# FumiyukiKato/FL-TEE

Hardware: AMD Instinct MI355X
Metric: aggregated params/sec (device-resident), 100 clients x MLP-MNIST updates (higher is better)
Workload: dtype f32; 1 GPU; ns: NS: baseline dense fp32 reduce, 100 clients x 1M params; alg=baseline, n_clients=100, d_per_gpu=1000000, k=1000000, record_bytes=8, parallelism=param-range shard x1

## Files before the change

### fl-tee_amd/csrc/common.h

```cpp
#pragma once
#include <hip/hip_runtime.h>
#include <stddef.h>
#include <stdint.h>
#include <stdlib.h>

#include "fltee_agg.h"
#include "rows.h"

__device__ __forceinline__ uint32_t rec_idx(uint64_t r) { return (uint32_t)r; }

constexpr uint32_t kSwzMask = 0x3FF0u;
__device__ __forceinline__ uint32_t swz_x(uint32_t p) {
    const uint32_t h = p >> 14;
    return ((h ^ (h >> 10)) << 4) & kSwzMask;
}
__device__ __forceinline__ uint32_t phys(uint32_t p) { return p ^ swz_x(p); }
__device__ __forceinline__ float rec_val(uint64_t r) { return __uint_as_float((uint32_t)(r >> 32)); }
__device__ __forceinline__ uint64_t make_rec(uint32_t idx, float val) {
    return ((uint64_t)__float_as_uint(val) << 32) | idx;
}

#define FLTEE_STREAM_DP 0x44504E5Au
#define FLTEE_STREAM_LAPLACE 0x4C41504Cu
#define FLTEE_STREAM_SAMPLE 0x534D504Cu

__host__ __device__ __forceinline__ uint32_t mix32(uint32_t x) {
    x ^= x >> 16;
    x *= 0x7feb352du;
    x ^= x >> 15;
    x *= 0x846ca68bu;
    x ^= x >> 16;
    return x;
}

__host__ __device__ __forceinline__ uint32_t shuffle_step_key(uint32_t seed, uint32_t ilog,
                                                              uint32_t jlog) {
    return mix32(mix32(seed) + ((ilog << 8) | jlog) * 0x9E3779B9u);
}

__host__ __device__ __forceinline__ void philox4x32_10(uint32_t c[4], uint32_t k0, uint32_t k1) {
#pragma unroll
    for (int r = 0; r < 10; ++r) {
        uint64_t p0 = (uint64_t)0xD2511F53u * c[0];
        uint64_t p1 = (uint64_t)0xCD9E8D57u * c[2];
        uint32_t n0 = (uint32_t)(p1 >> 32) ^ c[1] ^ k0;
        uint32_t n1 = (uint32_t)p1;
        uint32_t n2 = (uint32_t)(p0 >> 32) ^ c[3] ^ k1;
        uint32_t n3 = (uint32_t)p0;
        c[0] = n0; c[1] = n1; c[2] = n2; c[3] = n3;
        k0 += 0x9E3779B9u;
        k1 += 0xBB67AE85u;
    }
}

#define FLTEE_CHECK_LAUNCH(st)                                            \
    do {                                                                  \
        if (hipGetLastError() != hipSuccess) return FLTEE_ERROR_UNEXPECTED; \
    } while (0)

static inline size_t next_pow2_sz(size_t x) {
    size_t p = 1;
    while (p < x) p <<= 1;
    return p;
}
constexpr size_t kMaxNetRecords = (size_t)1 << 29;
static inline uint32_t log2_pow2(size_t x) {
    uint32_t l = 0;
    while (((size_t)1 << l) < x) ++l;
    return l;
}

namespace fltee {
bool trace_on();
void trace_event(const char *what, const char *site, uint64_t a, uint64_t b, uint64_t c);
}
#define FLTEE_LAUNCH(K, GRID, BLOCK, LDS, S, ...)                                              \
    do {                                                                                       \
        const dim3 fltee_g_ = dim3(GRID), fltee_b_ = dim3(BLOCK);                              \
        if (::fltee::trace_on())                                                               \
            ::fltee::trace_event("launch", #K, ((uint64_t)fltee_g_.x << 32) | fltee_g_.y,      \
                                 ((uint64_t)fltee_g_.z << 32) | fltee_b_.x, (uint64_t)(LDS));  \
        hipLaunchKernelGGL(K, fltee_g_, fltee_b_, LDS, S, __VA_ARGS__);                        \
    } while (0)
namespace fltee {
inline hipError_t fl_memcpy_async(void *d, const void *s, size_t n, hipMemcpyKind k, hipStream_t st) {
    if (trace_on()) trace_event("memcpy", "", n, (uint64_t)k, 0);
    return hipMemcpyAsync(d, s, n, k, st);
}
inline hipError_t fl_memcpy2d_async(void *d, size_t dp, const void *s, size_t sp, size_t w, size_t h,
                                    hipMemcpyKind k, hipStream_t st) {
    if (trace_on()) trace_event("memcpy2d", "", w, h, (uint64_t)k);
    return hipMemcpy2DAsync(d, dp, s, sp, w, h, k, st);
}
inline hipError_t fl_memcpy(void *d, const void *s, size_t n, hipMemcpyKind k) {
    if (trace_on()) trace_event("memcpy_sync", "", n, (uint64_t)k, 0);
    return hipMemcpy(d, s, n, k);
}
inline hipError_t fl_memset_async(void *d, int v, size_t n, hipStream_t st) {
    if (trace_on()) trace_event("memset", "", n, (uint64_t)(uint32_t)v, 0);
    return hipMemsetAsync(d, v, n, st);
}
inline hipError_t fl_memset(void *d, int v, size_t n) {
    if (trace_on()) trace_event("memset_sync", "", n, (uint64_t)(uint32_t)v, 0);
    return hipMemset(d, v, n);
}
inline hipError_t fl_stream_sync(hipStream_t st) {
    if (trace_on()) trace_event("sync", "stream", 0, 0, 0);
    return hipStreamSynchronize(st);
}
inline hipError_t fl_device_sync() {
    if (trace_on()) trace_event("sync", "device", 0, 0, 0);
    return hipDeviceSynchronize();
}
}

namespace fltee {

void net_account(uint64_t bytes, const char *kernel, hipStream_t s);

hipError_t launch_dense_accumulate(const void *rec, size_t n, size_t d, float coef, float *out,
                                   const float *client_coef, bool accumulate, uint32_t *status,
                                   hipStream_t s);
hipError_t launch_sweep_accumulate(const void *rec, size_t nrec, size_t d, float coef, float *out,
                                   bool accumulate, hipStream_t s);
hipError_t launch_scale(float *out, size_t d, float coef, hipStream_t s);
hipError_t launch_check_range(const void *rec, size_t nrec, uint32_t limit, uint32_t *status,
                              hipStream_t s);

hipError_t launch_dense_accumulate_rows(RowFmt fmt, const void *rows, size_t n, size_t d, float coef, float *out,
                                        const float *client_coef, bool accumulate, hipStream_t s);
hipError_t launch_rows_clip_coef(RowFmt fmt, const void *rows, size_t n, size_t d, float clipping, float *coef,
                                 hipStream_t s);
hipError_t launch_unpack_rows(RowFmt fmt, const void *rows, size_t n, size_t d, uint64_t *rec, hipStream_t s);
hipError_t launch_pack_rows(RowFmt fmt, const float *values, size_t n, size_t d, void *rows, hipStream_t s);

hipError_t launch_trimmed_mean(const void *in, bool packed, size_t n, size_t d, size_t t, float coef,
                               float *out, const float *client_coef, bool accumulate, uint32_t *status,
                               hipStream_t s);

hipError_t bitonic_sort(uint64_t *data, size_t m, uint32_t mode, uint32_t seed, hipStream_t s,
                        size_t valid = 0);
void set_pad_skip(int on);
void set_swizzle(int on);
bool pad_skip_enabled();
size_t debug_plan(uint32_t mlog, uint32_t tlog, uint32_t NT, int rmax, uint32_t *out, size_t cap);
void debug_pad_units(uint32_t mode, uint32_t valid, uint32_t mlog, uint32_t pbase, uint32_t ilog,
                     uint32_t jstep, uint32_t sblog, uint32_t uplog, uint32_t out[3]);
hipError_t bitonic_sort_segments(uint64_t *data, size_t m, size_t seg, uint32_t mode,
                                 hipStream_t s);
hipError_t bitonic_sort_advanced(uint64_t *data, size_t m, const void *rec, size_t nrec, size_t d,
                                 hipStream_t s);
hipError_t bitonic_sort_nips19(uint64_t *data, size_t m, uint32_t seed, const void *rec, size_t nrec,
                               const uint32_t *r, size_t d, size_t tf, hipStream_t s);
size_t bitonic_select_tiles(size_t m);
hipError_t bitonic_sort_nips19_select(uint64_t *data, size_t m, uint32_t seed, const void *rec,
                                      size_t nrec, const uint32_t *r, size_t d, size_t tf,
                                      uint32_t *tile_cnt, hipStream_t s);
void set_fused_init(int on);
hipError_t bitonic_sort_range(uint64_t *data, size_t m, uint32_t mode, uint32_t seed,
                              uint32_t pbase, hipStream_t s, uint32_t valid = 0);
hipError_t bitonic_merge_range(uint64_t *data, size_t m, uint32_t mode, uint32_t seed,
                               uint32_t ilog, uint32_t pbase, hipStream_t s);
hipError_t bitonic_steps_range(uint64_t *data, size_t m, uint32_t mode, uint32_t seed,
                               uint32_t ilog, uint32_t jtop, uint32_t jbot, uint32_t pbase,
                               hipStream_t s);
hipError_t bitonic_exchange(uint64_t *mine, const uint64_t *theirs, size_t m, uint32_t pos_mine,
                            uint32_t pos_theirs, uint32_t mode, uint32_t seed, uint32_t ilog,
                            uint32_t jlog, hipStream_t s);

size_t stable_sort_max_records();
hipError_t stable_sort(void *data16, size_t m, hipStream_t s, size_t valid = 0, bool init = false,
                       const void *rec = nullptr, size_t nrec = 0, size_t d = 0,
                       uint64_t *out8 = nullptr);
hipError_t stable_sort_range(void *data16, size_t m, size_t pos_base, hipStream_t s, size_t valid = 0,
                             bool init = false, const void *rec = nullptr, size_t nrec = 0,
                             size_t d = 0, uint64_t *out8 = nullptr);
hipError_t stable_merge_range(void *data16, size_t m, size_t pos_base, uint32_t stage, hipStream_t s,
                              uint64_t *out8 = nullptr);
hipError_t stable_exchange(void *mine16, const void *theirs16, size_t m, size_t pos_mine,
                           size_t pos_theirs, uint32_t stage, hipStream_t s);
hipError_t stable_init_range(const void *rec, size_t nrec, size_t d, size_t pos_base, size_t m,
                             void *dst16, hipStream_t s);
hipError_t stable_strip_range(const void *data16, size_t m, uint64_t *dst8, hipStream_t s);

hipError_t launch_advanced_init(const void *rec, size_t nrec, size_t d, size_t m, uint64_t *dst,
                                hipStream_t s);
hipError_t launch_advanced_init_range(const void *rec, size_t nrec, size_t d, size_t pbase,
                                      size_t m, uint64_t *dst, hipStream_t s);
size_t fold_context(size_t halo);
constexpr uint32_t kFsPiece = 1u, kFsFull = 2u, kFsCorr = 4u;
struct FoldSide {
    uint32_t F, K;
    float Q;
    uint32_t fl;
    uint32_t ck;
    float S;
    uint32_t pad[2];
};
struct FoldAgg {
    uint32_t F, K;
    float Q;
    uint32_t fl;
};
__device__ __forceinline__ FoldAgg fa_combine(const FoldAgg &x, const FoldAgg &y) {
    if (!(x.fl & kFsPiece)) return y;
    if (!(y.fl & kFsPiece)) return x;
    const bool yfull = (y.fl & kFsFull) != 0;
    FoldAgg r;
    r.F = x.F;
    r.K = y.K;
    r.fl = kFsPiece | (((x.fl & kFsFull) && yfull && x.K == y.F) ? kFsFull : 0u);
    r.Q = (yfull && y.F == x.K) ? __fadd_rn(x.Q, y.Q) : y.Q;
    return r;
}

__device__ __forceinline__ FoldAgg fa_of(const FoldSide &sd) {
    FoldAgg a;
    a.F = sd.F;
    a.K = sd.K;
    a.Q = sd.Q;
    a.fl = sd.fl & (kFsPiece | kFsFull);
    return a;
}

__device__ __forceinline__ FoldAgg fa_empty() {
    FoldAgg a;
    a.F = a.K = 0;
    a.Q = 0.0f;
    a.fl = 0;
    return a;
}

__host__ __device__ inline FoldAgg *fold_wave_aggs(FoldSide *side, size_t waves) {
    return reinterpret_cast<FoldAgg *>(side + waves * 64);
}
size_t fold_lanes(size_t span, size_t fold_len, size_t halo, size_t origin, long long pbase);
size_t fold_side_bytes(size_t span, size_t fold_len, size_t halo, size_t origin, long long pbase);
hipError_t launch_fold_range(const uint64_t *src, uint64_t *dst, size_t m, size_t origin,
                             size_t end, long long pbase, size_t fold_len, size_t halo,
                             FoldSide *side, hipStream_t s, size_t cemit_d = 0,
                             uint64_t cdummy = 0);
hipError_t launch_fold_range_total(const FoldSide *side, size_t lanes, FoldAgg *total,
                                   hipStream_t s);
hipError_t launch_fold_range_patch(uint64_t *dst, size_t span, size_t origin, long long pbase,
                                   size_t fold_len, size_t halo, const FoldSide *side,
                                   const FoldAgg *prev, size_t nprev, hipStream_t s,
                                   size_t cemit_d = 0, uint64_t cdummy = 0);
hipError_t launch_fold(const uint64_t *src, uint64_t *dst, size_t m, size_t fold_len, size_t halo,
                       void *side_ws, size_t side_cap, hipStream_t s, size_t cemit_d = 0,
                       uint64_t cdummy = 0);
hipError_t launch_extract(const uint64_t *src, size_t d, float coef, float *out, bool accumulate,
                          hipStream_t s);
size_t fc_lookback_bytes(size_t M, size_t L, size_t d, size_t halo);
hipError_t launch_fold_compact_extract(uint64_t *A, uint64_t *B, size_t M, size_t L, size_t d,
                                       size_t halo, float coef, float *out, bool accumulate,
                                       uint32_t *status, hipStream_t s, void *lb, size_t lb_cap,
                                       uint32_t *epoch);
hipError_t launch_compact_extract(uint64_t *src, uint64_t *tmp, size_t L, size_t d, float coef,
                                  float *out, bool accumulate, hipStream_t s);
uint64_t compact_dummy();
hipError_t launch_compact_extract_converted(uint64_t *src, uint64_t *tmp, size_t L, size_t d,
                                            float coef, float *out, bool accumulate, hipStream_t s);
hipError_t launch_compact_offset(const uint64_t *chunk, size_t c, size_t d, uint64_t *buf,
                                 uint64_t *tmp, float coef, float *out, hipStream_t s);
hipError_t launch_composite_init(const void *rec, size_t nrec, size_t d, size_t m, uint64_t *keys,
                                 uint32_t *status, hipStream_t s);

hipError_t launch_laplace_r(size_t d, size_t k, float T, uint64_t seed, uint32_t *r,
                            hipStream_t s);
hipError_t launch_nips19_build(const void *rec, size_t nrec, const uint32_t *r, size_t d,
                               size_t tf, size_t m, uint64_t *dst, hipStream_t s);
size_t select_tiles(size_t m);
hipError_t launch_select_count(const uint64_t *src, size_t m, size_t d, uint32_t *cnt,
                               uint32_t *base, hipStream_t s);
hipError_t launch_select_write(const uint64_t *src, size_t m, size_t d, const uint32_t *base,
                               uint64_t *dst, hipStream_t s);
hipError_t launch_select_scan(const uint32_t *cnt, size_t nb, uint32_t *base, hipStream_t s);
hipError_t launch_select_gather(const uint64_t *data, uint32_t tlog, size_t ntiles,
                                const uint32_t *cnt, const uint32_t *base, uint64_t *sel,
                                hipStream_t s);
hipError_t launch_nips19_build_range(const void *rec, size_t nrec, const uint32_t *r, size_t d,
                                     size_t tf, size_t pbase, size_t m, uint64_t *dst,
                                     hipStream_t s);

size_t radix_scratch_bytes(size_t n, size_t d);
hipError_t launch_sort_records_by_idx(const void *rec, size_t n, size_t d, void *scratch,
                                      size_t bytes, uint64_t *sorted, uint32_t *status,
                                      float *zero, size_t nzero, hipStream_t s);
hipError_t launch_fold_sorted(const uint64_t *sorted, size_t n, size_t d, float coef, float *out,
                              bool accumulate, hipStream_t s);
hipError_t launch_gather_by_keys(const uint64_t *keys, size_t n, const void *rec, uint64_t *dst,
                                 hipStream_t s);

size_t oram_slots(size_t d);
bool oram_supported(size_t d);
size_t oram_accesses(size_t nrec, size_t d, bool lazy);
bool oram_fits(size_t nrec, size_t d, bool lazy);
void set_oram_bucket(int z);
hipError_t launch_oram_tree(const void *rec, size_t nrec, size_t d, bool lazy, void *tree,
                            uint64_t seed, uint64_t *keys, uint64_t *keys2, uint64_t *records,
                            float coef, bool accumulate, float *out, uint32_t *status,
                            hipStream_t s);

hipError_t launch_dp_noise(float *out, size_t d, float sigma, float clipping, size_t n,
                           uint64_t seed, hipStream_t s);
hipError_t launch_client_clip_coef(const void *rec, size_t n, size_t k, float clipping,
                                   float *coef, hipStream_t s);
hipError_t launch_apply_clip(void *rec, size_t n, size_t k, const float *coef, hipStream_t s);

void aes128_expand_key(const uint8_t key[16], uint32_t rk[44]);
void aes128_session_round_keys(const uint32_t *ids, size_t n, uint32_t *rk);
hipError_t launch_aes_ctr(const uint8_t *cipher, size_t n, size_t bytes_per_client,
                          size_t rec_per_client, const uint32_t *round_keys, uint8_t *plain,
                          hipStream_t s, uint32_t *zero_word = nullptr);
void set_aes_variant(int v);
hipError_t launch_aes_ctr_slice(const uint8_t *cipher, size_t n, size_t bytes_per_client,
                                size_t rec_per_client, const uint32_t *round_keys, uint8_t *plain,
                                uint64_t block_off, uint32_t idx_sub, hipStream_t s,
                                uint32_t *zero_word = nullptr);
hipError_t launch_aes_ctr_gcm(const uint8_t *in, size_t n, size_t in_stride, size_t rec_per_client,
                              const uint32_t *round_keys, uint8_t *out, size_t out_stride,
                              const uint8_t iv[12], hipStream_t s, uint32_t *zero_word = nullptr);
hipError_t launch_aes_ctr_gcm_slice(const uint8_t *in, size_t n, size_t in_stride, size_t rec_per_client,
                                    const uint32_t *round_keys, uint8_t *out, size_t out_stride,
                                    const uint8_t iv[12], uint64_t first_block, uint32_t idx_sub,
                                    hipStream_t s);
void aes128_gcm_subkeys(const uint32_t *rk, size_t n, const uint8_t iv[12], uint8_t *sub);
void aes128_gcm_subkeys_portable(const uint32_t *rk, size_t n, const uint8_t iv[12], uint8_t *sub);
void aes128_session_round_keys_portable(const uint32_t *ids, size_t n, uint32_t *rk);
bool host_has_aesni();

size_t ghash_segments(size_t ct_bytes, size_t aad_len);
size_t ghash_pow_bytes(size_t n);
size_t ghash_part_bytes(size_t n, size_t ct_bytes, size_t aad_len);
hipError_t launch_ghash_powers(const uint8_t *sub, size_t n, void *pow, hipStream_t s);
hipError_t launch_ghash_bulk(const uint8_t *cipher, size_t n, size_t stride, size_t ct_bytes,
                             const uint8_t *aad, size_t aad_len, const void *pow, void *part,
                             hipStream_t s);
hipError_t launch_ghash_finish(uint8_t *cipher, size_t n, size_t stride, size_t ct_bytes,
                               size_t aad_len, const uint8_t *sub, const void *pow, const void *part,
                               bool emit, uint32_t *fail, uint32_t *status, hipStream_t s);
hipError_t launch_ghash_window(const uint8_t *window, size_t n, size_t stride, size_t ct_bytes,
                               uint64_t first_block, size_t win_bytes, const uint8_t *aad,
                               size_t aad_len, bool with_aad, const void *pow, void *part,
                               hipStream_t s);
hipError_t launch_ghash_merge(void *acc, const void *part, size_t n, size_t P, hipStream_t s);
hipError_t launch_ghash_finish_tags(uint8_t *tags, size_t tag_stride, size_t n, size_t ct_bytes,
                                    size_t aad_len, const uint8_t *sub, const void *pow,
                                    const void *part, bool emit, uint32_t *fail, uint32_t *status,
                                    hipStream_t s);
void ghash_window_host(const uint8_t h[16], const uint8_t *aad, size_t aad_len, bool with_aad,
                       const uint8_t *ct_window, size_t ct_bytes, uint64_t first_block,
                       size_t win_bytes, uint8_t *part_out);
bool gather_clients_fits(size_t n, size_t k, size_t n_keep);
hipError_t launch_gather_clients(const void *rec, size_t n, size_t k, const uint32_t *keep,
                                 size_t n_keep, void *out, uint32_t *status, hipStream_t s);

void gf128_mul_host(const uint8_t a[16], const uint8_t b[16], uint8_t out[16]);
void gcm_tag_host(const uint8_t h[16], const uint8_t ej0[16], const uint8_t *aad, size_t aad_len,
                  const uint8_t *ct, size_t ct_len, uint8_t tag[16]);

}
```

### fl-tee_amd/csrc/engine.h

```cpp
#pragma once
#include <mutex>
#include <vector>

#include "common.h"

namespace fltee {

constexpr int kMaxDevices = 64;

struct Buffer {
    void *ptr = nullptr;
    size_t cap = 0;
    uint32_t grow_bit = 0;
    bool reserve(size_t bytes);
    void release();
};

struct HostBuffer {
    void *ptr = nullptr;
    void *dptr = nullptr;
    size_t cap = 0;
    bool reserve(size_t bytes);
};

enum Ws { kWsA, kWsB, kWsMat, kWsR, kWsCoef, kWsRec, kWsKeys, kWsRadix, kWsOram, kWsSide,
          kWsLb, kWsS16, kWsCnt, kWsSel, kWsCount };

enum Route : uint32_t {
    kRouteNone,
    kRouteDense,
    kRouteScatterRows,
    kRouteCountingFold,
    kRouteFlatOrdered,
    kRouteSweep,
    kRouteTree,
    kRouteTreeLazy,
    kRouteAdvanced,
    kRouteBubble,
    kRouteOptimized,
    kRouteNips19,
    kRoutePacked,
    kRouteTrimDense,
    kRouteTrimPacked,
    kRouteBf16,
};
enum Tail : uint32_t {
    kTailNone,
    kTailFused,
    kTailStream,
    kTailOneEntry,
    kTailSort,
};

struct AdvShape {
    size_t nrec = 0, d = 0, L = 0, M = 0, fold_len = 0;
    size_t halo = 0;
    size_t span = 0;
    Tail tail = kTailNone;
    bool stable = false;
    size_t side_bytes = 0, lb_bytes = 0;
};

struct Plan {
    fltee_status_t status = FLTEE_SUCCESS;
    Route route = kRouteNone;
    bool clip_records = false;
    bool unpack = false;
    AdvShape adv;
    AdvShape adv_last;
    size_t batch = 0;
    size_t tree_slots = 0;
    size_t kq = 0, tf = 0, L = 0, M = 0;
    float T = 0.0f;
    size_t sel_tiles = 0;
    size_t bytes[kWsCount] = {};
};

struct DeviceCtx {
    bool ready = false;
    int device = -1;
    uint32_t *status = nullptr;
    Buffer ws_a, ws_b, ws_mat, ws_r, ws_coef, ws_rec;
    size_t mat_clean = 0, mat_clean_cap = 0;
    void *mat_clean_ptr = nullptr;
    Buffer cipher, records, round_keys, outbuf;
    Buffer stage;
    HostBuffer pin_in, pin_out;
    hipEvent_t call_ev[3] = {};
    Buffer gcm_sub, gcm_pow, gcm_part, gcm_fail;
    Buffer survivors;
    std::vector<uint32_t> keep_host;
    Buffer ws_client, ws_client_coef;
    Buffer ws_cnt, ws_sel;
    Buffer ws_keys, ws_radix;
    Buffer ws_oram;
    Buffer ws_side;
    Buffer ws_lb;
    Buffer ws_s16;
    uint32_t fc_epoch = 0;
    uint32_t *host_word = nullptr;
    hipStream_t stream = nullptr;
    hipStream_t copy_stream = nullptr;
    static constexpr int kCopyEvents = 64;
    hipEvent_t copy_ev[kCopyEvents] = {};
};

std::recursive_mutex &api_mutex();

DeviceCtx *device_ctx(int dev);
DeviceCtx *current_ctx();
uint64_t next_seed();
void set_debug_seed(uint64_t seed);
float nips19_threshold(size_t d, size_t k, size_t n);

void set_oram_tree(int on);
bool oram_tree_default();
void set_exact_runs(int on);
bool exact_runs_default();
void set_bubble_ecall(int on);
bool bubble_ecall_default();

fltee_status_t aggregate(uint32_t alg, const void *rec, size_t n, size_t k, size_t d, float *out,
                         const fltee_device_opts &o, hipStream_t s, uint32_t *status);
hipError_t safe_aggregate_ordered(DeviceCtx *c, const uint64_t *src, size_t m, size_t d,
                                  float coef, float *out, bool accumulate, uint32_t *status,
                                  hipStream_t s);
hipError_t ordered_from_list(DeviceCtx *c, const uint64_t *sel, size_t lc, size_t d, float coef,
                             float *out, bool acc, uint32_t *status, hipStream_t s);
hipError_t advanced_batch(const void *rec, size_t n, size_t k, size_t d, size_t halo, float *out,
                          uint32_t *status, hipStream_t s);
hipError_t read_device_word(DeviceCtx *c, const uint32_t *dev_word, size_t *out, hipStream_t s);
size_t workspace_bytes(uint32_t alg, size_t n, size_t k, size_t d, const fltee_device_opts &o);
bool reserve(uint32_t alg, size_t n, size_t k, size_t d, const fltee_device_opts &o);
fltee_status_t plan_status(uint32_t alg, size_t n, size_t k, size_t d, const fltee_device_opts &o);

}
```

### fl-tee_amd/csrc/engine.hip

```cpp
#include <sys/random.h>
#include <time.h>

#include <atomic>
#include <cmath>
#include <cstddef>
#include <cstdio>
#include <cstring>
#include <mutex>
#include <string>
#include <vector>

#include "common.h"
#include "engine.h"

namespace fltee {

hipError_t launch_rows_accumulate(const float *mat, size_t n, size_t d, float coef, float *out,
                                  bool accumulate, hipStream_t s);
hipError_t launch_scatter_sum(const void *rec, size_t n, size_t k, size_t d, uint32_t *mat,
                              size_t *mat_clean,
                              uint32_t *dup, float coef, float *out, bool accumulate,
                              uint32_t *status, hipStream_t s);

static bool use_scatter_rows(size_t n, size_t k, size_t d) {
    const size_t cells = n * d;
    return cells <= ((size_t)1 << 30) &&
           (cells <= ((size_t)1 << 24) || cells <= 64 * next_pow2_sz(n * k));
}

static bool flat_ordered(size_t n, size_t k, size_t d) { return k == d && n * k > 0; }

static Buffer DeviceCtx::*const kScratch[kWsCount] = {
    &DeviceCtx::ws_a,    &DeviceCtx::ws_b,    &DeviceCtx::ws_mat,   &DeviceCtx::ws_r,    &DeviceCtx::ws_coef,
    &DeviceCtx::ws_rec,  &DeviceCtx::ws_keys, &DeviceCtx::ws_radix, &DeviceCtx::ws_oram, &DeviceCtx::ws_side,
    &DeviceCtx::ws_lb,   &DeviceCtx::ws_s16,  &DeviceCtx::ws_cnt,   &DeviceCtx::ws_sel};
static std::atomic<uint32_t> g_scratch_grown{0};

static DeviceCtx g_ctx[kMaxDevices];
static std::mutex g_ctx_mu;
static std::atomic<uint64_t> g_debug_seed{0};
static std::atomic<uint64_t> g_seed_calls{0};

static std::atomic<uint64_t> g_net_launches{0}, g_net_bytes{0};
struct NetLaunch {
    const char *kernel;
    uint64_t bytes;
    hipEvent_t ev;
};
static std::mutex g_net_mu;
static std::vector<NetLaunch> g_net_log;
static std::atomic<bool> g_net_timing{false};
constexpr size_t kNetLogCap = 16384;

static std::atomic<bool> g_trace{false};
static std::mutex g_trace_mu;
static std::string g_trace_text;
static size_t g_trace_lines = 0;
constexpr size_t kTraceCap = (size_t)64 << 20;

bool trace_on() { return g_trace.load(std::memory_order_relaxed); }

void trace_event(const char *what, const char *site, uint64_t a, uint64_t b, uint64_t c) {
    char line[512];
    const int len = std::snprintf(line, sizeof line, "%s|%s|%llu|%llu|%llu\n", what, site,
                                  (unsigned long long)a, (unsigned long long)b, (unsigned long long)c);
    std::lock_guard<std::mutex> lk(g_trace_mu);
    if (len > 0 && g_trace_text.size() + (size_t)len < kTraceCap) {
        g_trace_text.append(line, (size_t)len < sizeof line ? (size_t)len : sizeof line - 1);
        ++g_trace_lines;
    }
}

void net_account(uint64_t bytes, const char *kernel, hipStream_t s) {
    if (trace_on()) trace_event("bytes", kernel, bytes, 0, 0);
    g_net_launches.fetch_add(1, std::memory_order_relaxed);
    g_net_bytes.fetch_add(bytes, std::memory_order_relaxed);
    if (!g_net_timing.load(std::memory_order_relaxed)) return;
    std::lock_guard<std::mutex> lk(g_net_mu);
    if (g_net_log.size() >= kNetLogCap) return;
    hipEvent_t e = nullptr;
    if (hipEventCreate(&e) != hipSuccess) return;
    if (hipEventRecord(e, s) != hipSuccess) { (void)hipEventDestroy(e); return; }
    g_net_log.push_back({kernel, bytes, e});
}

static void net_log_clear() {
    for (auto &r : g_net_log) (void)hipEventDestroy(r.ev);
    g_net_log.clear();
}

uint64_t next_seed() {
    const uint64_t s = g_debug_seed.load();
    if (s) return s + 0x9E3779B97F4A7C15ull * (++g_seed_calls);
    uint64_t r = 0;
    if (getrandom(&r, sizeof r, 0) != (ssize_t)sizeof r) r = (uint64_t)time(nullptr) * 0x2545F4914F6CDD1Dull;
    return r ? r : 1;
}

void set_debug_seed(uint64_t seed) {
    g_debug_seed.store(seed);
    g_seed_calls.store(0);
}

DeviceCtx *device_ctx(int dev) {
    if (dev < 0 || dev >= kMaxDevices) return nullptr;
    std::lock_guard<std::mutex> lk(g_ctx_mu);
    DeviceCtx &c = g_ctx[dev];
    if (!c.ready) {
        if (hipSetDevice(dev) != hipSuccess) return nullptr;
        if (hipMalloc(&c.status, 256) != hipSuccess) return nullptr;
        if (fl_memset(c.status, 0, 256) != hipSuccess) return nullptr;
        c.device = dev;
        for (int w = 0; w < kWsCount; ++w) (c.*kScratch[w]).grow_bit = 1u << w;
        c.ready = true;
    }
    return &c;
}

DeviceCtx *current_ctx() {
    int dev = 0;
    if (hipGetDevice(&dev) != hipSuccess) return nullptr;
    return device_ctx(dev);
}

bool Buffer::reserve(size_t bytes) {
    if (bytes <= cap) return true;
    g_scratch_grown.fetch_or(grow_bit, std::memory_order_relaxed);
    if (ptr) (void)hipFree(ptr);
    ptr = nullptr;
    cap = 0;
    const size_t want = bytes + bytes / 8 + 256;
    if (hipMalloc(&ptr, want) != hipSuccess) { ptr = nullptr; return false; }
    cap = want;
    return true;
}

bool HostBuffer::reserve(size_t bytes) {
    if (bytes <= cap) return true;
    if (ptr) (void)hipHostFree(ptr);
    ptr = dptr = nullptr;
    cap = 0;
    const size_t want = bytes + bytes / 8 + 4096;
    if (hipHostMalloc(&ptr, want, hipHostMallocDefault) != hipSuccess) { ptr = nullptr; return false; }
    if (hipHostGetDevicePointer(&dptr, ptr, 0) != hipSuccess) dptr = ptr;
    cap = want;
    return true;
}

void Buffer::release() {
    if (ptr) (void)hipFree(ptr);
    ptr = nullptr;
    cap = 0;
}

float nips19_threshold(size_t d, size_t k, size_t n) {
    const float epsilon = 100.0f, delta = 1.0f / (float)n;
    const float l1 = 2.0f * (float)k;
    return l1 / epsilon * logf((float)d / delta);
}

static size_t f32_to_usize_sat(float x) {
    if (!(x > 0.0f)) return 0;
    if (x >= 18446744073709551616.0f) return SIZE_MAX;
    return (size_t)x;
}

static bool g_radix_order = true;
static bool g_advanced_compaction = true;
static bool g_nips19_fused_select = true;
void set_radix_order(int on) { g_radix_order = on != 0; }

static size_t advanced_fold_span(size_t L, size_t M) {
    const size_t mf = (L + 1 + 15) / 16 * 16;
    return mf > M ? M : mf;
}

static size_t ordered_radix_bytes(size_t n, size_t d, bool network_order) {
    return g_radix_order && !network_order ? radix_scratch_bytes(n, d) : next_pow2_sz(n) * 8;
}

static AdvShape adv_shape(size_t n, size_t k, size_t d, size_t k_req, size_t halo) {
    AdvShape a;
    a.nrec = n * k, a.d = d, a.L = n * k + d, a.M = next_pow2_sz(a.L);
    a.fold_len = n * k_req + d, a.halo = halo ? halo : n, a.span = a.M;
    if (a.fold_len != a.L || !g_advanced_compaction) {
        a.tail = kTailSort;
    } else if ((a.lb_bytes = fc_lookback_bytes(a.M, a.L, d, a.halo)) != 0) {
        a.tail = kTailFused;
    } else {
        a.span = advanced_fold_span(a.L, a.M);
        a.tail = a.span >= 2 ? kTailStream : kTailOneEntry;
    }
    if (a.tail != kTailFused) a.side_bytes = fold_side_bytes(a.span, a.fold_len, a.halo, 0, 0);
    return a;
}

static void plan_adv_bytes(Plan &p, const AdvShape &a) {
    auto up = [&p](Ws w, size_t b) { if (b > p.bytes[w]) p.bytes[w] = b; };
    up(kWsA, a.M * 8), up(kWsB, a.M * 8), up(kWsSide, a.side_bytes), up(kWsLb, a.lb_bytes);
    if (a.stable) up(kWsS16, a.M * 16);
}

static RowFmt row_format(uint32_t flags) {
    return (flags & FLTEE_OPT_PACKED) ? kRowsF32 : (flags & FLTEE_OPT_BF16) ? kRowsBf16 : kRowsNone;
}

static Plan plan_for(uint32_t alg, size_t n, size_t k, size_t d, const fltee_device_opts &o) {
    Plan p;
    const RowFmt fmt = row_format(o.flags);
    const bool packed = fmt == kRowsF32, bf16 = fmt == kRowsBf16;
    const bool dense = fmt != kRowsNone || (o.flags & FLTEE_OPT_DENSE) != 0;
    const bool tree = alg == FLTEE_ALG_PATH_ORAM && (o.flags & FLTEE_OPT_ORAM_TREE);
    const bool trim = (o.flags & FLTEE_OPT_TRIM) != 0;
    const size_t nrec = n * k, k_req = (o.flags & FLTEE_OPT_K_REQ) ? o.k_req : k;
    auto refuse_if = [&p](bool bad) { if (bad) p.status = FLTEE_ERROR_INVALID_PARAMETER; };
    refuse_if(n == 0 || nrec + d >= ((size_t)1 << 31) || (dense && k != d) ||
              (fmt != kRowsNone && d < rows_min_d(fmt)) ||
              (o.flags & (FLTEE_OPT_PACKED | FLTEE_OPT_BF16)) == (FLTEE_OPT_PACKED | FLTEE_OPT_BF16));
    if (trim) {
        const bool flat = alg == FLTEE_ALG_BASELINE || alg == FLTEE_ALG_NON_OBLIVIOUS || alg == FLTEE_ALG_PATH_ORAM;
        refuse_if(!flat || !dense || (o.flags & (FLTEE_OPT_ORAM_TREE | FLTEE_OPT_ORAM_LAZY)) ||
                  o.trim > FLTEE_TRIM_MAX || 2 * o.trim >= n);
    }
    switch (alg) {
    case FLTEE_ALG_PATH_ORAM:
    case FLTEE_ALG_BASELINE:
    case FLTEE_ALG_NON_OBLIVIOUS:
        if (tree) {
            const bool lazy = (o.flags & FLTEE_OPT_ORAM_LAZY) != 0;
            p.route = lazy ? kRouteTreeLazy : kRouteTree;
            refuse_if(!oram_fits(nrec, d, lazy));
            p.tree_slots = oram_slots(d);
            p.bytes[kWsOram] = p.tree_slots * (lazy ? 24 : 16);
            p.bytes[kWsA] = p.bytes[kWsB] = next_pow2_sz(oram_accesses(nrec, d, lazy)) * 8;
            if (lazy) plan_adv_bytes(p, p.adv = adv_shape(1, p.tree_slots, d, p.tree_slots, 1));
        } else if (dense) {
            p.route = packed ? kRoutePacked : bf16 ? kRouteBf16 : kRouteDense;
            if (trim && o.trim) p.route = packed ? kRouteTrimPacked : kRouteTrimDense;
        } else if (alg == FLTEE_ALG_NON_OBLIVIOUS && use_scatter_rows(n, k, d)) {
            p.route = kRouteScatterRows;
            p.bytes[kWsMat] = n * d * 4;
        } else if (alg == FLTEE_ALG_NON_OBLIVIOUS || flat_ordered(n, k, d)) {
            const bool net = alg != FLTEE_ALG_NON_OBLIVIOUS;
            p.route = net ? kRouteFlatOrdered : kRouteCountingFold;
            refuse_if(next_pow2_sz(nrec) > kMaxNetRecords);
            p.bytes[kWsKeys] = nrec * 8, p.bytes[kWsRadix] = ordered_radix_bytes(nrec, d, net);
        } else {
            p.route = kRouteSweep;
        }
        break;
    case FLTEE_ALG_BUBBLE:
        p.route = kRouteBubble;
        p.adv = adv_shape(n, k, d, k, o.fold_halo);
        p.adv.stable = true;
        refuse_if(k_req != k || p.adv.M > kMaxNetRecords || p.adv.M > stable_sort_max_records());
        plan_adv_bytes(p, p.adv);
        break;
    case FLTEE_ALG_ADVANCED:
        p.route = kRouteAdvanced;
        p.adv = adv_shape(n, k, d, k_req, o.fold_halo);
        refuse_if(p.adv.M > kMaxNetRecords || p.adv.fold_len > p.adv.L);
        plan_adv_bytes(p, p.adv);
        break;
    case FLTEE_ALG_OPTIMIZED:
        p.route = kRouteOptimized;
        p.batch = o.batch && o.batch < n ? o.batch : n;
        p.adv = adv_shape(p.batch, k, d, k, o.fold_halo);
        refuse_if(p.adv.M > kMaxNetRecords);
        plan_adv_bytes(p, p.adv);
        if (p.batch && n % p.batch)
            plan_adv_bytes(p, p.adv_last = adv_shape(n % p.batch, k, d, k, o.fold_halo));
        break;
    case FLTEE_ALG_NIPS19:
        p.route = kRouteNips19;
        p.kq = k_req;
        p.T = nips19_threshold(d, p.kq, n);
        p.tf = f32_to_usize_sat(p.T);
        p.bytes[kWsR] = d * 4;
        refuse_if(p.tf > ((size_t)1 << 31) / (d ? d : 1));
        if (p.status != FLTEE_SUCCESS) break;
        p.L = nrec + d * p.tf, p.M = next_pow2_sz(p.L);
        refuse_if(p.M > kMaxNetRecords);
        p.bytes[kWsA] = p.M * 8;
        p.sel_tiles = g_nips19_fused_select && d ? bitonic_select_tiles(p.M) : 0;
        p.bytes[kWsCnt] = (2 * (p.sel_tiles > select_tiles(p.M) ? p.sel_tiles : select_tiles(p.M)) + 2) * 4;
        break;
    default:
        refuse_if(true);
        break;
    }
    if (o.flags & FLTEE_OPT_CLIP) {
        p.bytes[kWsCoef] = n * 4;
        p.clip_records = p.route != kRouteDense && p.route != kRoutePacked && p.route != kRouteTrimDense &&
                         p.route != kRouteTrimPacked && p.route != kRouteBf16;
        if (p.clip_records) p.bytes[kWsRec] = nrec * 8;
    }
    p.unpack = fmt != kRowsNone && p.route != kRoutePacked && p.route != kRouteTrimPacked && p.route != kRouteBf16;
    if (p.unpack) p.bytes[kWsRec] = nrec * 8;
    return p;
}

static bool reserve_lb(DeviceCtx *c, size_t bytes, const hipStream_t *s) {
    const bool grow = bytes > c->ws_lb.cap;
    if (!bytes || (!grow && (!s || c->fc_epoch < (1u << 30) - 1))) return true;
    if (!c->ws_lb.reserve(bytes)) return false;
    if ((s ? fl_memset_async(c->ws_lb.ptr, 0, c->ws_lb.cap, *s) : fl_memset(c->ws_lb.ptr, 0, c->ws_lb.cap)) !=
        hipSuccess)
        return false;
    c->fc_epoch = 0;
    return true;
}

static bool reserve_plan(DeviceCtx *c, const Plan &p, const hipStream_t *s) {
    for (int w = 0; w < kWsCount; ++w)
        if (!(w == kWsLb ? reserve_lb(c, p.bytes[w], s) : (c->*kScratch[w]).reserve(p.bytes[w]))) return false;
    return true;
}

static bool g_exact_runs = false;
void set_exact_runs(int on) { g_exact_runs = on != 0; }
bool exact_runs_default() { return g_exact_runs; }
static bool g_bubble_ecall = false;
void set_bubble_ecall(int on) { g_bubble_ecall = on != 0; }
bool bubble_ecall_default() { return g_bubble_ecall; }
static bool g_oram_tree = false;
void set_oram_tree(int on) { g_oram_tree = on != 0; }
bool oram_tree_default() { return g_oram_tree; }

static hipError_t ordered_fold_records(DeviceCtx *c, const void *rec, size_t n, size_t d,
                                       float coef, float *out, bool acc, uint32_t *status,
                                       hipStream_t s, bool network_order = false) {
    if (n == 0) return acc ? hipSuccess : fl_memset_async(out, 0, d * 4, s);
    uint64_t *sorted = (uint64_t *)c->ws_keys.ptr;
    hipError_t e;
    if (g_radix_order && !network_order) {
        e = launch_sort_records_by_idx(rec, n, d, c->ws_radix.ptr, c->ws_radix.cap, sorted, status,
                                       acc ? nullptr : out, d, s);
    } else {
        const size_t mc = next_pow2_sz(n);
        uint64_t *keys = (uint64_t *)c->ws_radix.ptr;
        e = launch_composite_init(rec, n, d, mc, keys, status, s);
        if (e == hipSuccess) e = bitonic_sort(keys, mc, 1, 0, s, n);
        if (e == hipSuccess) e = launch_gather_by_keys(keys, n, rec, sorted, s);
        if (e == hipSuccess && !acc) e = fl_memset_async(out, 0, d * 4, s);
    }
    if (e == hipSuccess) e = launch_fold_sorted(sorted, n, d, coef, out, acc, s);
    return e;
}

hipError_t ordered_from_list(DeviceCtx *c, const uint64_t *sel, size_t lc, size_t d, float coef,
                             float *out, bool acc, uint32_t *status, hipStream_t s) {
    if (lc && (!c->ws_keys.reserve(lc * 8) || !c->ws_radix.reserve(ordered_radix_bytes(lc, d, false))))
        return hipErrorOutOfMemory;
    return ordered_fold_records(c, sel, lc, d, coef, out, acc, status, s);
}

static hipError_t debug_sort_records(DeviceCtx *c, const void *rec, size_t n, size_t d, void *dst,
                                     uint32_t *status, hipStream_t s) {
    if (n == 0) return hipSuccess;
    if (!c->ws_keys.reserve(n * 8) || !c->ws_radix.reserve(ordered_radix_bytes(n, d, false)))
        return hipErrorOutOfMemory;
    uint64_t *sorted = (uint64_t *)c->ws_keys.ptr;
    hipError_t e;
    if (g_radix_order) {
        e = launch_sort_records_by_idx(rec, n, d, c->ws_radix.ptr, c->ws_radix.cap, sorted, status,
                                       nullptr, 0, s);
    } else {
        const size_t mc = next_pow2_sz(n);
        uint64_t *keys = (uint64_t *)c->ws_radix.ptr;
        e = launch_composite_init(rec, n, d, mc, keys, status, s);
        if (e == hipSuccess) e = bitonic_sort(keys, mc, 1, 0, s, n);
        if (e == hipSuccess) e = launch_gather_by_keys(keys, n, rec, sorted, s);
    }
    if (e == hipSuccess) e = fl_memcpy_async(dst, sorted, n * 8, hipMemcpyDeviceToDevice, s);
    return e;
}

hipError_t read_device_word(DeviceCtx *c, const uint32_t *dev_word, size_t *out, hipStream_t s) {
    if (!c->host_word && hipHostMalloc((void **)&c->host_word, 64, hipHostMallocDefault) != hipSuccess) {
        c->host_word = nullptr;
        return hipErrorOutOfMemory;
    }
    hipError_t e = fl_memcpy_async(c->host_word, dev_word, 4, hipMemcpyDeviceToHost, s);
    if (e == hipSuccess) e = fl_stream_sync(s);
    if (e == hipSuccess) *out = *c->host_word;
    return e;
}

hipError_t safe_aggregate_ordered(DeviceCtx *c, const uint64_t *src, size_t m, size_t d,
                                  float coef, float *out, bool acc, uint32_t *status,
                                  hipStream_t s) {
    if (d == 0) return hipSuccess;
    if (m == 0) return acc ? hipSuccess : fl_memset_async(out, 0, d * 4, s);
    const size_t nb = select_tiles(m);
    if (!c->ws_cnt.reserve((2 * nb + 2) * 4)) return hipErrorOutOfMemory;
    uint32_t *cnt = (uint32_t *)c->ws_cnt.ptr, *base = cnt + nb + 1;
    hipError_t e = launch_select_count(src, m, d, cnt, base, s);
    size_t lc = 0;
    if (e == hipSuccess) e = read_device_word(c, base + nb, &lc, s);
    if (e != hipSuccess) return e;
    if (!c->ws_sel.reserve(lc * 8 + 8)) return hipErrorOutOfMemory;
    uint64_t *sel = (uint64_t *)c->ws_sel.ptr;
    if (lc) e = launch_select_write(src, m, d, base, sel, s);
    if (e != hipSuccess) return e;
    return ordered_from_list(c, sel, lc, d, coef, out, acc, status, s);
}

static hipError_t nips19_shuffle_aggregate(DeviceCtx *c, const Plan &p, uint32_t key, const void *rec,
                                           size_t nrec, size_t d, float coef, float *out, bool acc,
                                           uint32_t *status, hipStream_t s) {
    const size_t ntl = p.sel_tiles;
    uint64_t *A = (uint64_t *)c->ws_a.ptr;
    uint32_t *cnt = (uint32_t *)c->ws_cnt.ptr, *base = cnt + ntl + 1;
    hipError_t e = fl_memset_async(cnt, 0, ntl * 4, s);
    if (e == hipSuccess)
        e = bitonic_sort_nips19_select(A, p.M, key, rec, nrec, (const uint32_t *)c->ws_r.ptr, d, p.tf, cnt, s);
    if (e != hipSuccess) return e;
    e = launch_select_scan(cnt, ntl, base, s);
    size_t lc = 0;
    if (e == hipSuccess) e = read_device_word(c, base + ntl, &lc, s);
    if (e != hipSuccess) return e;
    if (!c->ws_sel.reserve(lc * 8 + 8)) return hipErrorOutOfMemory;
    uint64_t *sel = (uint64_t *)c->ws_sel.ptr;
    if (lc) e = launch_select_gather(A, log2_pow2(p.M / ntl), ntl, cnt, base, sel, s);
    if (e != hipSuccess) return e;
    return ordered_from_list(c, sel, lc, d, coef, out, acc, status, s);
}

static hipError_t run_advanced(DeviceCtx *c, const void *rec, const AdvShape &a, float coef, float *out,
                               bool acc, uint32_t *status, hipStream_t s) {
    uint64_t *A = (uint64_t *)c->ws_a.ptr, *B = (uint64_t *)c->ws_b.ptr;
    hipError_t e;
    if (a.stable) {
        e = stable_sort(c->ws_s16.ptr, a.M, s, a.L, true, rec, a.nrec, a.d, A);
    } else {
        e = bitonic_sort_advanced(A, a.M, rec, a.nrec, a.d, s);
        if (e == hipErrorNotSupported) {
            e = launch_advanced_init(rec, a.nrec, a.d, a.M, A, s);
            if (e == hipSuccess) e = bitonic_sort(A, a.M, 0, 0, s, a.L);
        }
    }
    if (e != hipSuccess) return e;
    switch (a.tail) {
    case kTailFused:
        if (!reserve_lb(c, a.lb_bytes, &s)) return hipErrorOutOfMemory;
        return launch_fold_compact_extract(A, B, a.M, a.L, a.d, a.halo, coef, out, acc, status, s,
                                           c->ws_lb.ptr, c->ws_lb.cap, &c->fc_epoch);
    case kTailStream:
        e = launch_fold(A, B, a.span, a.fold_len, a.halo, c->ws_side.ptr, c->ws_side.cap, s, a.d,
                        compact_dummy());
        if (e != hipSuccess) return e;
        return launch_compact_extract_converted(B, A, a.L, a.d, coef, out, acc, s);
    case kTailOneEntry:
        e = launch_fold(A, B, a.span, a.fold_len, a.halo, c->ws_side.ptr, c->ws_side.cap, s);
        if (e != hipSuccess) return e;
        return launch_compact_extract(B, A, a.L, a.d, coef, out, acc, s);
    default:
        e = launch_fold(A, B, a.M, a.fold_len, a.halo, c->ws_side.ptr, c->ws_side.cap, s);
        if (e == hipSuccess) e = bitonic_sort(B, a.M, 0, 0, s, a.L);
        if (e == hipSuccess) e = launch_extract(B, a.d, coef, out, acc, s);
        return e;
    }
}

hipError_t advanced_batch(const void *rec, size_t n, size_t k, size_t d, size_t halo, float *out,
                          uint32_t *status, hipStream_t s) {
    DeviceCtx *c = current_ctx();
    if (!c) return hipErrorInvalidDevice;
    fltee_device_opts o;
    std::memset(&o, 0, sizeof o);
    o.fold_halo = halo;
    const Plan p = plan_for(FLTEE_ALG_ADVANCED, n, k, d, o);
    if (p.status != FLTEE_SUCCESS) return hipErrorInvalidValue;
    if (!reserve_plan(c, p, &s)) return hipErrorOutOfMemory;
    return run_advanced(c, rec, p.adv, 1.0f, out, false, status, s);
}

fltee_status_t aggregate(uint32_t alg, const void *rec, size_t n, size_t k, size_t d, float *out,
                         const fltee_device_opts &o, hipStream_t s, uint32_t *status) {
    DeviceCtx *c = current_ctx();
    if (!c) return FLTEE_ERROR_UNEXPECTED;
    const Plan p = plan_for(alg, n, k, d, o);
    if (p.status != FLTEE_SUCCESS) return p.status;
    if (!reserve_plan(c, p, &s)) return FLTEE_ERROR_OUT_OF_MEMORY;
    const bool acc = (o.flags & FLTEE_OPT_ACCUMULATE) != 0;
    const size_t n_avg = o.n_avg ? o.n_avg : (o.flags & FLTEE_OPT_TRIM) ? n - 2 * o.trim : n;
    const float coef = (o.flags & FLTEE_OPT_NO_AVERAGE) ? 1.0f : 1.0f / (float)n_avg;

    const RowFmt sent = row_format(o.flags), fmt = p.unpack ? kRowsNone : sent;
    if (p.unpack) {
        if (launch_unpack_rows(sent, rec, n, d, (uint64_t *)c->ws_rec.ptr, s) != hipSuccess)
            return FLTEE_ERROR_UNEXPECTED;
        rec = c->ws_rec.ptr;
    }

    const float *ccoef = nullptr;
    if (o.flags & FLTEE_OPT_CLIP) {
        float *cf = (float *)c->ws_coef.ptr;
        if ((fmt != kRowsNone ? launch_rows_clip_coef(fmt, rec, n, d, o.clipping, cf, s)
                              : launch_client_clip_coef(rec, n, k, o.clipping, cf, s)) != hipSuccess)
            return FLTEE_ERROR_UNEXPECTED;
        ccoef = cf;
        if (p.clip_records) {
            if ((!p.unpack &&
                 fl_memcpy_async(c->ws_rec.ptr, rec, n * k * 8, hipMemcpyDeviceToDevice, s) != hipSuccess) ||
                launch_apply_clip(c->ws_rec.ptr, n, k, cf, s) != hipSuccess)
                return FLTEE_ERROR_UNEXPECTED;
            rec = c->ws_rec.ptr;
        }
    }

    hipError_t e = hipSuccess;
    switch (p.route) {
    case kRouteTree:
    case kRouteTreeLazy: {
        const bool lazy = p.route == kRouteTreeLazy;
        uint8_t *tree = (uint8_t *)c->ws_oram.ptr;
        uint64_t *recs = lazy ? (uint64_t *)(tree + p.tree_slots * 16) : nullptr;
        const uint64_t seed = o.seed ? o.seed : next_seed();
        e = launch_check_range(rec, n * k, (uint32_t)next_pow2_sz(d), status, s);
        if (e == hipSuccess)
            e = launch_oram_tree(rec, n * k, d, lazy, tree, seed, (uint64_t *)c->ws_a.ptr,
                                 (uint64_t *)c->ws_b.ptr, recs, coef, acc, out, status, s);
        if (e == hipSuccess && lazy) e = run_advanced(c, recs, p.adv, coef, out, acc, status, s);
        break;
    }
    case kRouteDense:
        e = launch_dense_accumulate(rec, n, d, coef, out, ccoef, acc, status, s);
        break;
    case kRoutePacked:
    case kRouteBf16:
        e = launch_dense_accumulate_rows(fmt, rec, n, d, coef, out, ccoef, acc, s);
        break;
    case kRouteTrimDense:
    case kRouteTrimPacked:
        e = launch_trimmed_mean(rec, p.route == kRouteTrimPacked, n, d, o.trim, coef, out, ccoef, acc, status, s);
        break;
    case kRouteScatterRows:
        if (c->mat_clean_ptr != c->ws_mat.ptr || c->mat_clean_cap != c->ws_mat.cap) {
            c->mat_clean = 0;
            c->mat_clean_ptr = c->ws_mat.ptr;
            c->mat_clean_cap = c->ws_mat.cap;
        }
        e = launch_scatter_sum(rec, n, k, d, (uint32_t *)c->ws_mat.ptr, &c->mat_clean,
                               c->status + 16, coef, out, acc, status, s);
        if (e != hipSuccess) c->mat_clean = 0;
        break;
    case kRouteCountingFold:
        e = ordered_fold_records(c, rec, n * k, d, coef, out, acc, status, s);
        break;
    case kRouteFlatOrdered:
    case kRouteSweep:
        if (alg == FLTEE_ALG_PATH_ORAM)
            e = launch_check_range(rec, n * k, (uint32_t)next_pow2_sz(d), status, s);
        if (e == hipSuccess && p.route == kRouteFlatOrdered)
            e = ordered_fold_records(c, rec, n * k, d, coef, out, acc, c->status + 32, s, true);
        else if (e == hipSuccess)
            e = launch_sweep_accumulate(rec, n * k, d, coef, out, acc, s);
        break;
    case kRouteAdvanced:
    case kRouteBubble:
        e = run_advanced(c, rec, p.adv, coef, out, acc, status, s);
        break;
    case kRouteOptimized:
        if (!acc) e = fl_memset_async(out, 0, d * 4, s);
        for (size_t c0 = 0; e == hipSuccess && c0 < n; c0 += p.batch)
            e = run_advanced(c, (const uint8_t *)rec + c0 * k * 8, c0 + p.batch <= n ? p.adv : p.adv_last,
                             1.0f, out, true, status, s);
        if (e == hipSuccess && !acc && coef != 1.0f) e = launch_scale(out, d, coef, s);
        break;
    case kRouteNips19: {
        const uint64_t seed = o.seed ? o.seed : next_seed();
        uint64_t *A = (uint64_t *)c->ws_a.ptr;
        const uint32_t *r = (const uint32_t *)c->ws_r.ptr;
        e = launch_laplace_r(d, p.kq, p.T, seed, (uint32_t *)c->ws_r.ptr, s);
        const uint32_t key = (uint32_t)(seed ^ (seed >> 32));
        bool done = false;
        if (e == hipSuccess && p.sel_tiles) {
            e = nips19_shuffle_aggregate(c, p, key, rec, n * k, d, coef, out, acc, status, s);
            done = e != hipErrorNotSupported;
            if (!done) e = hipSuccess;
        }
        if (e == hipSuccess && !done) {
            e = bitonic_sort_nips19(A, p.M, key, rec, n * k, r, d, p.tf, s);
            if (e == hipErrorNotSupported) {
                e = launch_nips19_build(rec, n * k, r, d, p.tf, p.M, A, s);
                if (e == hipSuccess) e = bitonic_sort(A, p.M, 2, key, s, p.L);
            }
            if (e == hipSuccess) e = safe_aggregate_ordered(c, A, p.M, d, coef, out, acc, status, s);
        }
        break;
    }
    default:
        return FLTEE_ERROR_INVALID_PARAMETER;
    }
    if (e == hipSuccess && (o.flags & FLTEE_OPT_DP)) {
        const uint64_t seed = o.seed ? o.seed : next_seed();
        e = launch_dp_noise(out, d, o.sigma, o.clipping, n_avg, seed, s);
    }
    if (e != hipSuccess)
        std::fprintf(stderr, "[fltee] aggregate(alg %u, n %zu, k %zu, d %zu): %s\n", alg, n, k, d,
                     hipGetErrorString(e));
    return e == hipSuccess ? FLTEE_SUCCESS : FLTEE_ERROR_UNEXPECTED;
}

size_t workspace_bytes(uint32_t alg, size_t n, size_t k, size_t d, const fltee_device_opts &o) {
    const Plan p = plan_for(alg, n, k, d, o);
    size_t sum = 0;
    for (size_t b : p.bytes) sum += b;
    return sum;
}

fltee_status_t plan_status(uint32_t alg, size_t n, size_t k, size_t d, const fltee_device_opts &o) {
    return plan_for(alg, n, k, d, o).status;
}

bool reserve(uint32_t alg, size_t n, size_t k, size_t d, const fltee_device_opts &o) {
    DeviceCtx *c = current_ctx();
    return c && reserve_plan(c, plan_for(alg, n, k, d, o), nullptr);
}

fltee_status_t debug_plan_words(uint32_t alg, size_t n, size_t k, size_t d, const fltee_device_opts &o,
                                uint64_t *out) {
    const Plan p = plan_for(alg, n, k, d, o);
    out[0] = p.route, out[1] = p.adv.tail;
    out[2] = p.route == kRouteNips19 ? p.M : p.adv.M, out[3] = p.adv.halo;
    for (int w = 0; w < kWsCount; ++w) out[4 + w] = p.bytes[w];
    return p.status;
}

void release_scratch() {
    DeviceCtx *c = current_ctx();
    if (!c) return;
    for (auto w : kScratch) (c->*w).release();
    c->mat_clean = c->mat_clean_cap = 0;
    c->mat_clean_ptr = nullptr;
    c->fc_epoch = 0;
}


}

using namespace fltee;

static fltee_device_opts default_opts() {
    fltee_device_opts o;
    std::memset(&o, 0, sizeof o);
    return o;
}

static fltee_device_opts read_opts(const fltee_device_opts *opts) {
    fltee_device_opts o = default_opts();
    if (!opts) return o;
    std::memcpy(&o, opts, offsetof(fltee_device_opts, trim));
    if (o.flags & FLTEE_OPT_TRIM) o.trim = opts->trim;
    return o;
}

extern "C" fltee_status_t fltee_aggregate_device(uint32_t alg, const void *d_records, size_t n,
                                                 size_t k, size_t d, float *d_out,
                                                 const fltee_device_opts *opts, void *stream) {
    std::lock_guard<std::recursive_mutex> lk(api_mutex());
    const fltee_device_opts o = read_opts(opts);
    if ((o.flags & FLTEE_OPT_BF16) && ((uintptr_t)d_records & 1)) return FLTEE_ERROR_INVALID_PARAMETER;
    DeviceCtx *c = current_ctx();
    if (!c) return FLTEE_ERROR_UNEXPECTED;
    uint32_t *status = o.d_status ? o.d_status : c->status;
    hipStream_t s = (hipStream_t)stream;
    if (!o.d_status && fl_memset_async(c->status, 0, 4, s) != hipSuccess) return FLTEE_ERROR_UNEXPECTED;
    return aggregate(alg, d_records, n, k, d, d_out, o, s, status);
}

extern "C" size_t fltee_workspace_bytes(uint32_t alg, size_t n, size_t k, size_t d,
                                        const fltee_device_opts *opts) {
    const fltee_device_opts o = read_opts(opts);
    return workspace_bytes(alg, n, k, d, o);
}

extern "C" fltee_status_t fltee_reserve(uint32_t alg, size_t n, size_t k, size_t d,
                                        const fltee_device_opts *opts) {
    std::lock_guard<std::recursive_mutex> lk(api_mutex());
    const fltee_device_opts o = read_opts(opts);
    if ((o.flags & FLTEE_OPT_TRIM) && plan_status(alg, n, k, d, o) != FLTEE_SUCCESS)
        return FLTEE_ERROR_INVALID_PARAMETER;
    return reserve(alg, n, k, d, o) ? FLTEE_SUCCESS : FLTEE_ERROR_OUT_OF_MEMORY;
}

extern "C" fltee_status_t fltee_device_status(void *stream, uint32_t *status) {
    std::lock_guard<std::recursive_mutex> lk(api_mutex());
    DeviceCtx *c = current_ctx();
    if (!c || !status) return FLTEE_ERROR_UNEXPECTED;
    hipStream_t s = (hipStream_t)stream;
    if (fl_stream_sync(s) != hipSuccess) return FLTEE_ERROR_UNEXPECTED;
    if (fl_memcpy(status, c->status, 4, hipMemcpyDeviceToHost) != hipSuccess)
        return FLTEE_ERROR_UNEXPECTED;
    if (fl_memset(c->status, 0, 4) != hipSuccess) return FLTEE_ERROR_UNEXPECTED;
    return FLTEE_SUCCESS;
}

extern "C" fltee_status_t fltee_bitonic_device(void *d_records, size_t m, uint32_t mode,
                                               uint32_t seed, void *stream) {
    if (m & (m - 1)) return FLTEE_ERROR_INVALID_PARAMETER;
    if (m >= ((size_t)1 << 31)) return FLTEE_ERROR_INVALID_PARAMETER;
    return bitonic_sort((uint64_t *)d_records, m, mode, seed, (hipStream_t)stream) == hipSuccess
               ? FLTEE_SUCCESS
               : FLTEE_ERROR_UNEXPECTED;
}

extern "C" fltee_status_t fltee_stable_sort_device(void *d_records16, size_t m, void *stream) {
    if (m == 0 || (m & (m - 1)) || m > stable_sort_max_records()) return FLTEE_ERROR_INVALID_PARAMETER;
    return stable_sort(d_records16, m, (hipStream_t)stream) == hipSuccess ? FLTEE_SUCCESS
                                                                          : FLTEE_ERROR_UNEXPECTED;
}

extern "C" fltee_status_t fltee_fold_device(const void *d_src, void *d_dst, size_t m,
                                            size_t fold_len, size_t halo, uint32_t *d_status,
                                            void *stream) {
    if (fold_len == 0 || fold_len > m || !d_status) return FLTEE_ERROR_INVALID_PARAMETER;
    std::lock_guard<std::recursive_mutex> lk(api_mutex());
    DeviceCtx *c = current_ctx();
    if (!c || !c->ws_side.reserve(fold_side_bytes(m, fold_len, halo, 0, 0)))
        return FLTEE_ERROR_OUT_OF_MEMORY;
    return launch_fold((const uint64_t *)d_src, (uint64_t *)d_dst, m, fold_len, halo,
                       c->ws_side.ptr, c->ws_side.cap, (hipStream_t)stream) == hipSuccess
               ? FLTEE_SUCCESS
               : FLTEE_ERROR_INVALID_PARAMETER;
}

extern "C" fltee_status_t fltee_laplace_r_device(size_t d, size_t k, size_t n, uint64_t seed,
                                                 uint32_t *d_r, float *T_out, void *stream) {
    if (n == 0) return FLTEE_ERROR_INVALID_PARAMETER;
    const float T = nips19_threshold(d, k, n);
    if (T_out) *T_out = T;
    return launch_laplace_r(d, k, T, seed, d_r, (hipStream_t)stream) == hipSuccess
               ? FLTEE_SUCCESS
               : FLTEE_ERROR_UNEXPECTED;
}

static bool range_ok(size_t m, size_t pos_base) {
    return m >= 2 && !(m & (m - 1)) && pos_base % m == 0 && pos_base + m <= ((size_t)1 << 31);
}

extern "C" fltee_status_t fltee_advanced_init_range_device(const void *d_records, size_t nrec,
                                                           size_t d, size_t pos_base, size_t m,
                                                           void *d_dst, void *stream) {
    return launch_advanced_init_range(d_records, nrec, d, pos_base, m, (uint64_t *)d_dst,
                                      (hipStream_t)stream) == hipSuccess
               ? FLTEE_SUCCESS
               : FLTEE_ERROR_UNEXPECTED;
}

extern "C" fltee_status_t fltee_bitonic_range_sort_device(void *d_records, size_t m,
                                                          size_t pos_base, uint32_t mode,
                                                          uint32_t seed, void *stream) {
    if (!range_ok(m, pos_base)) return FLTEE_ERROR_INVALID_PARAMETER;
    return bitonic_sort_range((uint64_t *)d_records, m, mode, seed, (uint32_t)pos_base,
                              (hipStream_t)stream) == hipSuccess
               ? FLTEE_SUCCESS
               : FLTEE_ERROR_UNEXPECTED;
}

extern "C" fltee_status_t fltee_bitonic_range_sort_padded_device(void *d_records, size_t m,
                                                                 size_t pos_base, size_t valid,
                                                                 uint32_t mode, uint32_t seed,
                                                                 void *stream) {
    if (!range_ok(m, pos_base)) return FLTEE_ERROR_INVALID_PARAMETER;
    if (valid == 0) return FLTEE_SUCCESS;
    return bitonic_sort_range((uint64_t *)d_records, m, mode, seed, (uint32_t)pos_base,
                              (hipStream_t)stream, valid >= m ? 0u : (uint32_t)valid) == hipSuccess
               ? FLTEE_SUCCESS
               : FLTEE_ERROR_UNEXPECTED;
}

extern "C" fltee_status_t fltee_bitonic_range_merge_device(void *d_records, size_t m,
                                                           size_t pos_base, uint32_t mode,
                                                           uint32_t seed, uint32_t stage_log,
                                                           void *stream) {
    if (!range_ok(m, pos_base) || ((size_t)1 << stage_log) <= m || stage_log > 31)
        return FLTEE_ERROR_INVALID_PARAMETER;
    return bitonic_merge_range((uint64_t *)d_records, m, mode, seed, stage_log,
                               (uint32_t)pos_base, (hipStream_t)stream) == hipSuccess
               ? FLTEE_SUCCESS
               : FLTEE_ERROR_UNEXPECTED;
}

extern "C" fltee_status_t fltee_bitonic_range_exchange_device(void *d_mine, const void *d_theirs,
                                                              size_t m, size_t pos_mine,
                                                              size_t pos_theirs, uint32_t mode,
                                                              uint32_t seed, uint32_t stage_log,
                                                              void *stream) {
    if (!range_ok(m, pos_mine) || !range_ok(m, pos_theirs) || stage_log > 31)
        return FLTEE_ERROR_INVALID_PARAMETER;
    const size_t j = pos_mine > pos_theirs ? pos_mine - pos_theirs : pos_theirs - pos_mine;
    if ((j & (j - 1)) || j < m || j >= ((size_t)1 << stage_log) || (pos_mine ^ pos_theirs) != j)
        return FLTEE_ERROR_INVALID_PARAMETER;
    return bitonic_exchange((uint64_t *)d_mine, (const uint64_t *)d_theirs, m, (uint32_t)pos_mine,
                            (uint32_t)pos_theirs, mode, seed, stage_log, log2_pow2(j),
                            (hipStream_t)stream) == hipSuccess
               ? FLTEE_SUCCESS
               : FLTEE_ERROR_UNEXPECTED;
}

extern "C" fltee_status_t fltee_bitonic_range_steps_device(void *d_records, size_t m,
                                                           size_t pos_base, uint32_t mode,
                                                           uint32_t seed, uint32_t stage_log,
                                                           uint32_t step_top, uint32_t step_bot,
                                                           void *stream) {
    if (!range_ok(m, pos_base) || stage_log > 31 || step_bot > step_top ||
        step_top >= stage_log || ((size_t)1 << step_top) >= m)
        return FLTEE_ERROR_INVALID_PARAMETER;
    return bitonic_steps_range((uint64_t *)d_records, m, mode, seed, stage_log, step_top,
                               step_bot, (uint32_t)pos_base, (hipStream_t)stream) == hipSuccess
               ? FLTEE_SUCCESS
               : FLTEE_ERROR_UNEXPECTED;
}

static bool stable_range_ok(size_t m, size_t pos_base) {
    return m >= ((size_t)1 << 12) && m <= ((size_t)1 << 29) && !(m & (m - 1)) && pos_base % m == 0 &&
           pos_base <= ((size_t)1 << 31) && pos_base + m <= ((size_t)1 << 31);
}

extern "C" fltee_status_t fltee_stable_init_range_device(const void *d_records, size_t nrec, size_t d,
                                                         size_t pos_base, size_t m, void *d_dst16,
                                                         void *stream) {
    if (!stable_range_ok(m, pos_base) || nrec >= ((size_t)1 << 31) || d >= ((size_t)1 << 31) ||
        nrec + d >= ((size_t)1 << 31))
        return FLTEE_ERROR_INVALID_PARAMETER;
    return stable_init_range(d_records, nrec, d, pos_base, m, d_dst16, (hipStream_t)stream) == hipSuccess
               ? FLTEE_SUCCESS
               : FLTEE_ERROR_UNEXPECTED;
}

extern "C" fltee_status_t fltee_stable_range_sort_device(void *d_rec16, size_t m, size_t pos_base,
                                                         size_t valid, void *stream) {
    if (!stable_range_ok(m, pos_base)) return FLTEE_ERROR_INVALID_PARAMETER;
    if (valid == 0) return FLTEE_SUCCESS;
    return stable_sort_range(d_rec16, m, pos_base, (hipStream_t)stream, valid >= m ? 0 : valid) ==
                   hipSuccess
               ? FLTEE_SUCCESS
               : FLTEE_ERROR_UNEXPECTED;
}

extern "C" fltee_status_t fltee_stable_range_exchange_device(void *d_mine16, const void *d_theirs16,
                                                             size_t m, size_t pos_mine,
                                                             size_t pos_theirs, uint32_t stage_log,
                                                             void *stream) {
    if (!stable_range_ok(m, pos_mine) || !stable_range_ok(m, pos_theirs) || pos_mine == pos_theirs ||
        stage_log > 31)
        return FLTEE_ERROR_INVALID_PARAMETER;
    const size_t j = pos_mine > pos_theirs ? pos_mine - pos_theirs : pos_theirs - pos_mine;
    if ((j & (j - 1)) || j >= ((size_t)1 << stage_log) || (pos_mine ^ pos_theirs) != j)
        return FLTEE_ERROR_INVALID_PARAMETER;
    return stable_exchange(d_mine16, d_theirs16, m, pos_mine, pos_theirs, stage_log,
                           (hipStream_t)stream) == hipSuccess
               ? FLTEE_SUCCESS
               : FLTEE_ERROR_UNEXPECTED;
}

extern "C" fltee_status_t fltee_stable_range_merge_device(void *d_rec16, size_t m, size_t pos_base,
                                                          uint32_t stage_log, void *stream) {
    if (!stable_range_ok(m, pos_base) || stage_log > 31 || ((size_t)1 << stage_log) <= m)
        return FLTEE_ERROR_INVALID_PARAMETER;
    return stable_merge_range(d_rec16, m, pos_base, stage_log, (hipStream_t)stream) == hipSuccess
               ? FLTEE_SUCCESS
               : FLTEE_ERROR_UNEXPECTED;
}

extern "C" fltee_status_t fltee_stable_range_strip_device(const void *d_rec16, size_t m, void *d_dst8,
                                                          void *stream) {
    if (!stable_range_ok(m, 0)) return FLTEE_ERROR_INVALID_PARAMETER;
    return stable_strip_range(d_rec16, m, (uint64_t *)d_dst8, (hipStream_t)stream) == hipSuccess
               ? FLTEE_SUCCESS
               : FLTEE_ERROR_UNEXPECTED;
}

extern "C" size_t fltee_fold_context(size_t halo) { return fold_context(halo); }

extern "C" size_t fltee_fold_side_bytes(size_t span, size_t halo) {
    return fold_side_bytes(span, (size_t)1 << 62, halo, 1, 1);
}

extern "C" fltee_status_t fltee_fold_range_device(const void *d_src, void *d_dst, size_t m,
                                                  size_t origin, size_t end, int64_t pos_base,
                                                  size_t fold_len, size_t halo, void *d_side,
                                                  void *stream) {
    if (!d_side || origin < fold_context(halo) + 1 || end > m || origin >= end || (origin & 1) ||
        (end & 1) || (m & 1))
        return FLTEE_ERROR_INVALID_PARAMETER;
    if (end < m ? false : (int64_t)end + pos_base < (int64_t)fold_len)
        return FLTEE_ERROR_INVALID_PARAMETER;
    return launch_fold_range((const uint64_t *)d_src, (uint64_t *)d_dst, m, origin, end,
                             (long long)pos_base, fold_len, halo, (FoldSide *)d_side,
                             (hipStream_t)stream) == hipSuccess
               ? FLTEE_SUCCESS
               : FLTEE_ERROR_UNEXPECTED;
}

extern "C" fltee_status_t fltee_fold_range_total_device(const void *d_side, size_t span,
                                                        size_t halo, void *d_total, void *stream) {
    if (!d_side || !d_total) return FLTEE_ERROR_INVALID_PARAMETER;
    const size_t lanes = fold_lanes(span, (size_t)1 << 62, halo, 1, 1);
    return launch_fold_range_total((const FoldSide *)d_side, lanes, (FoldAgg *)d_total,
                                   (hipStream_t)stream) == hipSuccess
               ? FLTEE_SUCCESS
               : FLTEE_ERROR_UNEXPECTED;
}

extern "C" fltee_status_t fltee_fold_range_patch_device(void *d_dst, size_t origin, size_t end,
                                                        int64_t pos_base, size_t fold_len,
                                                        size_t halo, const void *d_side,
                                                        const void *d_prev_totals, size_t n_prev,
                                                        void *stream) {
    if (!d_dst || !d_side || origin >= end || (n_prev && !d_prev_totals))
        return FLTEE_ERROR_INVALID_PARAMETER;
    return launch_fold_range_patch((uint64_t *)d_dst, end - origin, origin, (long long)pos_base,
                                   fold_len, halo, (const FoldSide *)d_side,
                                   (const FoldAgg *)d_prev_totals, n_prev, (hipStream_t)stream) ==
                   hipSuccess
               ? FLTEE_SUCCESS
               : FLTEE_ERROR_UNEXPECTED;
}

extern "C" fltee_status_t fltee_compact_range_device(const void *d_chunk, size_t c, size_t d,
                                                     void *d_buf, void *d_tmp, float coef,
                                                     float *d_out, void *stream) {
    if (d + c >= ((size_t)1 << 29)) return FLTEE_ERROR_INVALID_PARAMETER;
    return launch_compact_offset((const uint64_t *)d_chunk, c, d, (uint64_t *)d_buf,
                                 (uint64_t *)d_tmp, coef, d_out, (hipStream_t)stream) == hipSuccess
               ? FLTEE_SUCCESS
               : FLTEE_ERROR_UNEXPECTED;
}

extern "C" fltee_status_t fltee_nips19_build_range_device(const void *d_records, size_t nrec,
                                                          const uint32_t *d_r, size_t d,
                                                          size_t tf, size_t pos_base, size_t m,
                                                          void *d_dst, void *stream) {
    if (nrec + d * tf >= ((size_t)1 << 31)) return FLTEE_ERROR_INVALID_PARAMETER;
    return launch_nips19_build_range(d_records, nrec, d_r, d, tf, pos_base, m, (uint64_t *)d_dst,
                                     (hipStream_t)stream) == hipSuccess
               ? FLTEE_SUCCESS
               : FLTEE_ERROR_UNEXPECTED;
}

extern "C" fltee_status_t fltee_safe_aggregate_device(const void *d_src, size_t m, size_t d,
                                                      float *d_out, void *stream) {
    std::lock_guard<std::recursive_mutex> lk(api_mutex());
    DeviceCtx *c = current_ctx();
    if (!c) return FLTEE_ERROR_UNEXPECTED;
    if (m >= ((size_t)1 << 31)) return FLTEE_ERROR_INVALID_PARAMETER;
    return safe_aggregate_ordered(c, (const uint64_t *)d_src, m, d, 1.0f, d_out, false, c->status,
                                  (hipStream_t)stream) == hipSuccess
               ? FLTEE_SUCCESS
               : FLTEE_ERROR_UNEXPECTED;
}

extern "C" fltee_status_t fltee_select_device(const void *d_src, size_t m, size_t d, void *d_list,
                                              size_t cap, size_t *count, void *stream) {
    std::lock_guard<std::recursive_mutex> lk(api_mutex());
    DeviceCtx *c = current_ctx();
    if (!c || !count || m >= ((size_t)1 << 31)) return FLTEE_ERROR_INVALID_PARAMETER;
    hipStream_t s = (hipStream_t)stream;
    *count = 0;
    if (m == 0 || d == 0) return FLTEE_SUCCESS;
    const size_t nb = select_tiles(m);
    if (!c->ws_cnt.reserve((2 * nb + 2) * 4)) return FLTEE_ERROR_OUT_OF_MEMORY;
    uint32_t *cnt = (uint32_t *)c->ws_cnt.ptr, *base = cnt + nb + 1;
    size_t lc = 0;
    if (launch_select_count((const uint64_t *)d_src, m, d, cnt, base, s) != hipSuccess ||
        read_device_word(c, base + nb, &lc, s) != hipSuccess)
        return FLTEE_ERROR_UNEXPECTED;
    *count = lc;
    if (lc > cap || (lc && !d_list)) return FLTEE_ERROR_INVALID_PARAMETER;
    if (lc && launch_select_write((const uint64_t *)d_src, m, d, base, (uint64_t *)d_list, s) != hipSuccess)
        return FLTEE_ERROR_UNEXPECTED;
    return FLTEE_SUCCESS;
}

extern "C" fltee_status_t fltee_ordered_list_device(const void *d_list, size_t lc, size_t d,
                                                    float coef, float *d_out, void *stream) {
    std::lock_guard<std::recursive_mutex> lk(api_mutex());
    DeviceCtx *c = current_ctx();
    if (!c || lc >= ((size_t)1 << 29)) return FLTEE_ERROR_INVALID_PARAMETER;
    if (d == 0) return FLTEE_SUCCESS;
    return ordered_from_list(c, (const uint64_t *)d_list, lc, d, coef, d_out, false, c->status,
                             (hipStream_t)stream) == hipSuccess
               ? FLTEE_SUCCESS
               : FLTEE_ERROR_UNEXPECTED;
}

extern "C" fltee_status_t fltee_debug_sort_records_device(const void *d_rec, size_t n, size_t d,
                                                          void *d_sorted, void *stream) {
    std::lock_guard<std::recursive_mutex> lk(api_mutex());
    DeviceCtx *c = current_ctx();
    if (!c || d == 0 || n >= ((size_t)1 << 29) || (n && (!d_rec || !d_sorted)))
        return FLTEE_ERROR_INVALID_PARAMETER;
    return debug_sort_records(c, d_rec, n, d, d_sorted, c->status, (hipStream_t)stream) == hipSuccess
               ? FLTEE_SUCCESS
               : FLTEE_ERROR_UNEXPECTED;
}

extern "C" void fltee_debug_set_seed(uint64_t seed) { set_debug_seed(seed); }

extern "C" void fltee_debug_trace(int on) {
    std::lock_guard<std::mutex> lk(fltee::g_trace_mu);
    if (on) {
        fltee::g_trace_text.clear();
        fltee::g_trace_lines = 0;
    }
    fltee::g_trace.store(on != 0);
}

extern "C" size_t fltee_debug_trace_text(char *buf, size_t cap) {
    std::lock_guard<std::mutex> lk(fltee::g_trace_mu);
    const std::string &t = fltee::g_trace_text;
    if (buf && cap) {
        const size_t n = t.size() < cap - 1 ? t.size() : cap - 1;
        std::memcpy(buf, t.data(), n);
        buf[n] = 0;
    }
    return t.size();
}

extern "C" size_t fltee_debug_network_plan(uint32_t mlog, uint32_t tlog, uint32_t nt, int rmax,
                                           uint32_t *out, size_t cap) {
    return fltee::debug_plan(mlog, tlog, nt, rmax, out, cap);
}

extern "C" void fltee_debug_pad_units(uint32_t mode, uint32_t valid, uint32_t mlog, uint32_t pbase,
                                      uint32_t ilog, uint32_t jstep, uint32_t sblog, uint32_t uplog,
                                      uint32_t *out) {
    fltee::debug_pad_units(mode, valid, mlog, pbase, ilog, jstep, sblog, uplog, out);
}

extern "C" void fltee_debug_net_stats(uint64_t *launches, uint64_t *bytes, int reset) {
    if (launches) *launches = fltee::g_net_launches.load();
    if (bytes) *bytes = fltee::g_net_bytes.load();
    if (reset) {
        fltee::g_net_launches.store(0);
        fltee::g_net_bytes.store(0);
    }
}

extern "C" void fltee_debug_net_timing(int on, void *stream) {
    std::lock_guard<std::mutex> lk(fltee::g_net_mu);
    if (on) {
        fltee::net_log_clear();
        fltee::g_net_timing.store(true);
        return;
    }
    fltee::g_net_timing.store(false);
    hipEvent_t e = nullptr;
    if (hipEventCreate(&e) == hipSuccess) {
        if (hipEventRecord(e, (hipStream_t)stream) == hipSuccess)
            fltee::g_net_log.push_back({nullptr, 0, e});
        else
            (void)hipEventDestroy(e);
    }
}

extern "C" size_t fltee_debug_net_log(size_t i, char *name, size_t name_cap, uint64_t *bytes,
                                      float *ms) {
    std::lock_guard<std::mutex> lk(fltee::g_net_mu);
    const auto &L = fltee::g_net_log;
    const size_t nl = L.empty() ? 0 : (L.back().kernel ? L.size() : L.size() - 1);
    if (i < nl) {
        if (name && name_cap) {
            std::snprintf(name, name_cap, "%s", L[i].kernel ? L[i].kernel : "");
        }
        if (bytes) *bytes = L[i].bytes;
        if (ms) {
            *ms = -1.0f;
            if (i + 1 < L.size()) (void)hipEventElapsedTime(ms, L[i].ev, L[i + 1].ev);
        }
    }
    return nl;
}

extern "C" size_t fltee_packed_slice_bytes(size_t d) { return row_units(kRowsF32, d) * 8; }

extern "C" fltee_status_t fltee_unpack_dense_device(const void *d_packed, size_t n, size_t d,
                                                    void *d_records, void *stream) {
    if (n == 0 || d == 0 || d > 0xFFFFFFFFull || !d_packed || !d_records)
        return FLTEE_ERROR_INVALID_PARAMETER;
    return launch_unpack_rows(kRowsF32, d_packed, n, d, (uint64_t *)d_records, (hipStream_t)stream) == hipSuccess
               ? FLTEE_SUCCESS
               : FLTEE_ERROR_UNEXPECTED;
}

extern "C" fltee_status_t fltee_client_pack_dense_device(const float *d_values, size_t n, size_t d,
                                                         void *d_packed, void *stream) {
    if (n == 0 || d == 0 || d > 0xFFFFFFFFull || !d_values || !d_packed)
        return FLTEE_ERROR_INVALID_PARAMETER;
    return launch_pack_rows(kRowsF32, d_values, n, d, d_packed, (hipStream_t)stream) == hipSuccess
               ? FLTEE_SUCCESS
               : FLTEE_ERROR_UNEXPECTED;
}

extern "C" size_t fltee_bf16_slice_bytes(size_t d) { return row_units(kRowsBf16, d) * 8; }

extern "C" fltee_status_t fltee_unpack_bf16_device(const void *d_rows, size_t n, size_t d, void *d_records,
                                                   void *stream) {
    if (n == 0 || d == 0 || d > 0xFFFFFFFFull || !d_rows || !d_records || ((uintptr_t)d_rows & 1))
        return FLTEE_ERROR_INVALID_PARAMETER;
    return launch_unpack_rows(kRowsBf16, d_rows, n, d, (uint64_t *)d_records, (hipStream_t)stream) == hipSuccess
               ? FLTEE_SUCCESS
               : FLTEE_ERROR_UNEXPECTED;
}

extern "C" fltee_status_t fltee_client_pack_bf16_device(const float *d_values, size_t n, size_t d,
                                                        void *d_rows, void *stream) {
    if (n == 0 || d == 0 || d > 0xFFFFFFFFull || !d_values || !d_rows || ((uintptr_t)d_rows & 1))
        return FLTEE_ERROR_INVALID_PARAMETER;
    return launch_pack_rows(kRowsBf16, d_values, n, d, d_rows, (hipStream_t)stream) == hipSuccess
               ? FLTEE_SUCCESS
               : FLTEE_ERROR_UNEXPECTED;
}

extern "C" fltee_status_t fltee_sum_rows_device(const float *d_rows, size_t nrows, size_t d,
                                                float coef, float *d_out, void *stream) {
    if (nrows == 0) return FLTEE_ERROR_INVALID_PARAMETER;
    return launch_rows_accumulate(d_rows, nrows, d, coef, d_out, false, (hipStream_t)stream) ==
                   hipSuccess
               ? FLTEE_SUCCESS
               : FLTEE_ERROR_UNEXPECTED;
}

extern "C" fltee_status_t fltee_dp_noise_device(float *d_out, size_t d, float sigma,
                                                float clipping, size_t n, uint64_t seed,
                                                void *stream) {
    if (n == 0) return FLTEE_ERROR_INVALID_PARAMETER;
    return launch_dp_noise(d_out, d, sigma, clipping, n, seed ? seed : next_seed(),
                           (hipStream_t)stream) == hipSuccess
               ? FLTEE_SUCCESS
               : FLTEE_ERROR_UNEXPECTED;
}

namespace fltee {
void set_dense_variant(int v); void set_compact_variant(int v); void set_fold_compact(int on);
bool fold_compact_geometry(size_t M, size_t L, size_t d, size_t halo, uint64_t out[7]);
bool fold_stream_geometry(size_t span, size_t fold_len, size_t halo, uint64_t out[5]);
hipError_t launch_read_floor(const void *src, size_t bytes, uint32_t *sink, unsigned blocks, hipStream_t s);
}
extern "C" int fltee_debug_read_floor(const void *d_src, size_t bytes, void *d_sink, unsigned blocks,
                                      void *stream) {
    return fltee::launch_read_floor(d_src, bytes, (uint32_t *)d_sink, blocks, (hipStream_t)stream) ==
                   hipSuccess ? 0 : 1;
}
extern "C" void fltee_debug_set_dense_variant(int v) { fltee::set_dense_variant(v); }
extern "C" void fltee_debug_set_advanced_compaction(int on) { fltee::g_advanced_compaction = on != 0; }
extern "C" void fltee_debug_set_compact_variant(int v) { fltee::set_compact_variant(v); }
extern "C" void fltee_debug_set_fold_compact(int on) { fltee::set_fold_compact(on); }
extern "C" void fltee_debug_set_pad_skip(int on) { fltee::set_pad_skip(on); }
extern "C" void fltee_debug_set_radix_order(int on) { fltee::set_radix_order(on); }
extern "C" void fltee_set_path_oram_tree(int on) {
    std::lock_guard<std::recursive_mutex> lk(fltee::api_mutex());
    fltee::set_oram_tree(on);
}
extern "C" void fltee_set_advanced_exact_runs(int on) {
    std::lock_guard<std::recursive_mutex> lk(fltee::api_mutex());
    fltee::set_exact_runs(on);
}
extern "C" void fltee_set_bubble_ecall(int on) {
    std::lock_guard<std::recursive_mutex> lk(fltee::api_mutex());
    fltee::set_bubble_ecall(on);
}
extern "C" void fltee_debug_set_oram_bucket(int z) {
    std::lock_guard<std::recursive_mutex> lk(fltee::api_mutex());
    fltee::set_oram_bucket(z);
}
extern "C" void fltee_debug_set_aes_variant(int v) {
    std::lock_guard<std::recursive_mutex> lk(fltee::api_mutex());
    fltee::set_aes_variant(v);
}
extern "C" void fltee_debug_set_swizzle(int on) { fltee::set_swizzle(on); }
extern "C" void fltee_debug_set_fused_init(int on) { fltee::set_fused_init(on); }
extern "C" fltee_status_t fltee_debug_plan(uint32_t alg, size_t n, size_t k, size_t d,
                                           const fltee_device_opts *opts, uint64_t *out) {
    return fltee::debug_plan_words(alg, n, k, d, read_opts(opts), out);
}
extern "C" uint32_t fltee_debug_scratch_grown(void) { return fltee::g_scratch_grown.exchange(0); }
extern "C" void fltee_debug_scratch_release(void) {
    std::lock_guard<std::recursive_mutex> lk(fltee::api_mutex());
    fltee::release_scratch();
}
extern "C" void fltee_debug_fold_geometry(size_t M, size_t L, size_t d, size_t halo, uint64_t *out) {
    for (int i = 0; i < 8; ++i) out[i] = 0;
    if (fltee::g_advanced_compaction && fltee::fold_compact_geometry(M, L, d, halo, out + 1)) {
        out[0] = 1;
        return;
    }
    const size_t span = fltee::g_advanced_compaction ? fltee::advanced_fold_span(L, M) : M;
    out[0] = fltee::fold_stream_geometry(span, L, halo, out + 1) ? 2 : 3;
    out[6] = span;
}
extern "C" void fltee_debug_set_nips19_fused_select(int on) { fltee::g_nips19_fused_select = on != 0; }
extern "C" fltee_status_t fltee_debug_sort_fused(uint32_t gen, void *d_data, size_t m,
                                                 const void *d_rec, size_t nrec, const uint32_t *d_r,
                                                 size_t d, size_t tf, uint32_t seed, void *stream) {
    if (!d_data || (nrec && !d_rec) || (gen == 2 && d && tf && !d_r)) return FLTEE_ERROR_INVALID_PARAMETER;
    hipError_t e;
    if (gen == 1) e = fltee::bitonic_sort_advanced((uint64_t *)d_data, m, d_rec, nrec, d, (hipStream_t)stream);
    else if (gen == 2)
        e = fltee::bitonic_sort_nips19((uint64_t *)d_data, m, seed, d_rec, nrec, d_r, d, tf, (hipStream_t)stream);
    else return FLTEE_ERROR_INVALID_PARAMETER;
    if (e == hipErrorNotSupported || e == hipErrorInvalidValue) return FLTEE_ERROR_INVALID_PARAMETER;
    return e == hipSuccess ? FLTEE_SUCCESS : FLTEE_ERROR_UNEXPECTED;
}
```

### fl-tee_amd/csrc/k_compact.hip

```cpp
#include "common.h"

namespace fltee {


constexpr uint64_t CP_DUMMY = 0x80000000ull;
constexpr uint64_t CP_PAD = 0xFFFFFFFFull;

__device__ __forceinline__ uint64_t cp_pick(uint64_t self, uint64_t right, uint32_t j) {
    const uint32_t cs = (uint32_t)self, cr = (uint32_t)right;
    uint32_t lo, hi, e, em;
    const uint32_t dmy = 0x80000000u;
    asm("v_bfe_i32 %2, %4, %8, 1\n\t"
        "v_bfe_i32 %3, %6, %8, 1\n\t"
        "v_bfi_b32 %0, %2, %9, %4\n\t"
        "v_bfi_b32 %0, %3, %6, %0\n\t"
        "v_bfi_b32 %1, %3, %7, %5"
        : "=&v"(lo), "=&v"(hi), "=&v"(e), "=&v"(em)
        : "v"(cs), "v"((uint32_t)(self >> 32)), "v"(cr), "v"((uint32_t)(right >> 32)), "s"(j),
          "s"(dmy));
    return ((uint64_t)hi << 32) | lo;
}

__device__ __forceinline__ float cp_out(uint64_t r) { return ((uint32_t)r >> 31) ? 0.0f : rec_val(r); }

typedef unsigned int cp_u32x2 __attribute__((ext_vector_type(2)));
typedef unsigned int cp_u32x4 __attribute__((ext_vector_type(4)));

template <int NT, int PER, int G, int LW, int SH, int G0 = 0>
__device__ __forceinline__ void cp_levels_ct(uint64_t *sm, uint32_t j0, uint32_t t) {
    if constexpr (G0 < G) {
        constexpr bool two = G0 + 1 < G;
        constexpr uint32_t stepf = (1u << LW) << G0;
        constexpr uint32_t gl = two ? G0 + 1 : G0;
        constexpr uint32_t lim = ((uint32_t)SH - ((2u << gl) - 1)) << LW;
        const uint32_t j = j0 + (uint32_t)G0;
        uint64_t *const base = sm + t;
        uint64_t nv[PER];
#pragma unroll
        for (int i = 0; i < PER; ++i) {
            const uint32_t o = (uint32_t)i * NT;
            if (o + NT <= lim || t + o < lim) {
                if constexpr (two) {
                    const uint64_t y0 = cp_pick(base[o], base[o + stepf], j);
                    const uint64_t y2 = cp_pick(base[o + 2 * stepf], base[o + 3 * stepf], j);
                    nv[i] = cp_pick(y0, y2, j + 1);
                } else {
                    nv[i] = cp_pick(base[o], base[o + stepf], j);
                }
            }
        }
        __syncthreads();
#pragma unroll
        for (int i = 0; i < PER; ++i) {
            const uint32_t o = (uint32_t)i * NT;
            if (o + NT <= lim || t + o < lim) base[o] = nv[i];
        }
        __syncthreads();
        cp_levels_ct<NT, PER, G, LW, SH, G0 + (two ? 2 : 1)>(sm, j0, t);
    }
}

template <int NT, int PER, bool FIRST, int FINAL, int MINB = 1, bool V2 = false, int CG = 0, int CLW = 0,
          int CSH = 0, bool NH = false>
__global__ __launch_bounds__(NT, MINB) void compact_pass(const uint64_t *__restrict__ src,
                                                   uint64_t *__restrict__ dst, uint32_t L,
                                                   uint32_t d, uint32_t j0, uint32_t G,
                                                   uint32_t logW, uint32_t S, uint32_t rows,
                                                   uint32_t ngroups, float coef,
                                                   float *__restrict__ out, uint32_t ntiles) {
    constexpr uint32_t CAP = (uint32_t)NT * PER;
    __shared__ uint64_t sm[CAP];
    const uint32_t W = 1u << logW, H = (1u << G) - 1;
    auto tid = [] {
        uint32_t x = threadIdx.x;
        asm volatile("; compact tid" : "+v"(x));
        return x;
    };
    const __amdgpu_buffer_rsrc_t rs =
        __builtin_amdgcn_make_buffer_rsrc((void *)src, (short)0, (int)(L * 8u), 0x00020000);
    uint32_t tile = blockIdx.x;
    if (tile >= ntiles) return;
    auto pos_of = [&](uint32_t tl, uint32_t f) -> uint64_t {
        const uint32_t band = tl / ngroups, grp = tl - band * ngroups;
        return ((uint64_t)(band * S + (f >> logW)) << j0) + (grp << logW) + (f & (W - 1));
    };
    static_assert(!V2 || (!FIRST && PER % 2 == 0), "V2: strided passes, slot pairs");
    auto slot = [&](uint32_t i) -> uint32_t {
        return V2 ? 2u * (tid() + (i >> 1) * NT) + (i & 1u) : tid() + i * NT;
    };
    uint64_t pf[PER];
    const uint32_t used = (NH ? S : S + H) << logW;
    const uint32_t oob = L * 8u;
    auto prefetch = [&](uint32_t tl) {
        if constexpr (V2) {
#pragma unroll
            for (uint32_t i = 0; i < PER; i += 2) {
                const uint64_t p = pos_of(tl, slot(i));
                const cp_u32x4 x = __builtin_amdgcn_raw_buffer_load_b128(
                    rs, (int)(p < L && slot(i) < used ? (uint32_t)p * 8u : oob), 0, 0);
                pf[i] = ((uint64_t)x.y << 32) | x.x;
                pf[i + 1] = ((uint64_t)x.w << 32) | x.z;
            }
        } else {
#pragma unroll
            for (uint32_t i = 0; i < PER; ++i) {
                const uint64_t p = pos_of(tl, tid() + i * NT);
                const cp_u32x2 x = __builtin_amdgcn_raw_buffer_load_b64(
                    rs, (int)(p < L && tid() + i * NT < used ? (uint32_t)p * 8u : oob), 0, 0);
                pf[i] = ((uint64_t)x.y << 32) | x.x;
            }
        }
    };
    prefetch(tile);
    for (;;) {
#pragma unroll
        for (uint32_t i = 0; i < PER; ++i) {
            uint64_t v = pos_of(tile, slot(i)) < L ? pf[i] : CP_DUMMY;
            if (FIRST) {
                const uint32_t p = (uint32_t)pos_of(tile, tid() + i * NT), idx = (uint32_t)v;
                v = (v & 0xFFFFFFFF00000000ull) | (idx < d ? (uint64_t)(p - idx) : CP_DUMMY);
            }
            sm[slot(i)] = v;
        }
        __syncthreads();
        const uint32_t next = tile + gridDim.x;
        if (next < ntiles) prefetch(next);
        if constexpr (CG != 0) {
            cp_levels_ct<NT, PER, CG, CLW, CSH>(sm, j0, tid());
        } else {
        uint64_t nv[PER];
        auto rdl = [&](uint32_t x) -> uint64_t { return (!NH || x < used) ? sm[x] : CP_DUMMY; };
        for (uint32_t g = 0; g < G;) {
            const uint32_t stepf = W << g;
            const uint32_t j = j0 + g;
            const bool two = g + 1 < G;
            const uint32_t gl = two ? g + 1 : g;
            const uint32_t lim0 = (S + H - ((2u << gl) - 1)) << logW;
            const uint32_t lim = NH && used < lim0 ? used : lim0;
            if (two) {
#pragma unroll
                for (uint32_t i = 0; i < PER; ++i) {
                    const uint32_t f = tid() + i * NT;
                    if (f < lim) {
                        const uint64_t y0 = cp_pick(rdl(f), rdl(f + stepf), j);
                        const uint64_t y2 = cp_pick(rdl(f + 2 * stepf), rdl(f + 3 * stepf), j);
                        nv[i] = cp_pick(y0, y2, j + 1);
                    }
                }
            } else {
#pragma unroll
                for (uint32_t i = 0; i < PER; ++i) {
                    const uint32_t f = tid() + i * NT;
                    if (f < lim) nv[i] = cp_pick(rdl(f), rdl(f + stepf), j);
                }
            }
            __syncthreads();
#pragma unroll
            for (uint32_t i = 0; i < PER; ++i) {
                const uint32_t f = tid() + i * NT;
                if (f < lim) sm[f] = nv[i];
            }
            __syncthreads();
            g += two ? 2 : 1;
        }
        }
        const uint32_t nout = S << logW;
        if constexpr (V2 && FINAL == 0) {
            const __amdgpu_buffer_rsrc_t ds =
                __builtin_amdgcn_make_buffer_rsrc((void *)dst, (short)0, (int)(L * 8u), 0x00020000);
#pragma unroll
            for (uint32_t i = 0; i < PER; i += 2) {
                const uint32_t f = slot(i);
                if (f < nout) {
                    const uint64_t p = pos_of(tile, f);
                    const uint64_t a = sm[f], b = sm[f + 1];
                    const cp_u32x4 x = {(uint32_t)a, (uint32_t)(a >> 32), (uint32_t)b, (uint32_t)(b >> 32)};
                    __builtin_amdgcn_sched_barrier(0);
                    __builtin_amdgcn_raw_buffer_store_b128(x, ds, (int)(p < L ? (uint32_t)p * 8u : L * 8u), 0, 0);
                    __builtin_amdgcn_sched_barrier(0);
                    asm volatile("s_nop 1" ::: "memory");
                    __builtin_amdgcn_sched_barrier(0);
                }
            }
        } else {
#pragma unroll
        for (uint32_t i = 0; i < PER; ++i) {
            const uint32_t f = tid() + i * NT;
            if (f < nout) {
                const uint64_t p = pos_of(tile, f);
                if (FINAL == 0) {
                    if (p < L) dst[p] = sm[f];
                } else if (p < d) {
                    const float v = cp_out(sm[f]);
                    out[p] = FINAL == 2 ? __fadd_rn(out[p], v) : __fmul_rn(v, coef);
                }
            }
        }
        }
        if (next >= ntiles) break;
        __syncthreads();
        tile = next;
    }
}

constexpr int kCompactBlocks = 4;
constexpr int kCompactFirstBlocks = 4;
static int g_compact_variant = 1;
void set_compact_variant(int v) { g_compact_variant = v; }

constexpr uint32_t kCpTailMerge = 21;
template <int NT, int PER, int MINB = 1>
static hipError_t launch_pass(bool first, int fin, unsigned grid, hipStream_t s, const uint64_t *src,
                              uint64_t *dst, uint32_t L, uint32_t d, uint32_t j0, uint32_t G,
                              uint32_t logW, uint32_t S, uint32_t rows, uint32_t ngroups,
                              float coef, float *out, uint32_t ntiles, bool nh = false) {
#define CP_GO(F, X, V)                                                                           \
    FLTEE_LAUNCH((compact_pass<NT, PER, F, X, MINB, V>), dim3(grid), dim3(NT), 0, s, src, dst, L, \
                       d, j0, G, logW, S, rows, ngroups, coef, out, ntiles)
#define CP_GO_CT(V, G_, LW_, SH_)                                                                \
    FLTEE_LAUNCH((compact_pass<NT, PER, false, 0, MINB, V, G_, LW_, SH_>), dim3(grid), dim3(NT), 0, s, \
                       src, dst, L, d, j0, G, logW, S, rows, ngroups, coef, out, ntiles)
    const bool v2 = !first && (logW >= 1 || S % 2 == 0) && L % 2 == 0 &&
                    (uintptr_t)src % 16 == 0 && (uintptr_t)dst % 16 == 0;
    const uint32_t sh = S + (1u << G) - 1;
    if constexpr (NT * PER == 4096) {
        if (!first && v2 && fin == 0) {
            if (G == 9 && logW == 0 && sh == 4095) { CP_GO_CT(true, 9, 0, 4095); return hipGetLastError(); }
            if (G == 5 && logW == 4 && sh == 256) { CP_GO_CT(true, 5, 4, 256); return hipGetLastError(); }
        }
    }
#define CP_GO_NH(X, V)                                                                           \
    FLTEE_LAUNCH((compact_pass<NT, PER, false, X, MINB, V, 0, 0, 0, true>), dim3(grid), dim3(NT), 0, s, \
                       src, dst, L, d, j0, G, logW, S, rows, ngroups, coef, out, ntiles)
    if (nh && !first) {
        if (v2) {
            if (fin == 0) CP_GO_NH(0, true); else if (fin == 1) CP_GO_NH(1, true); else CP_GO_NH(2, true);
        } else {
            if (fin == 0) CP_GO_NH(0, false); else if (fin == 1) CP_GO_NH(1, false); else CP_GO_NH(2, false);
        }
        return hipGetLastError();
    }
#undef CP_GO_NH
    if (first) {
        if (fin == 0) CP_GO(true, 0, false); else if (fin == 1) CP_GO(true, 1, false); else CP_GO(true, 2, false);
    } else if (v2) {
        if (fin == 0) CP_GO(false, 0, true); else if (fin == 1) CP_GO(false, 1, true); else CP_GO(false, 2, true);
    } else {
        if (fin == 0) CP_GO(false, 0, false); else if (fin == 1) CP_GO(false, 1, false); else CP_GO(false, 2, false);
    }
#undef CP_GO
#undef CP_GO_CT
    return hipGetLastError();
}

static uint32_t bitlen(uint64_t x) {
    uint32_t b = 0;
    while (x) { ++b; x >>= 1; }
    return b;
}

static hipError_t compact_levels(uint64_t *src, uint64_t *tmp, size_t L, size_t d,
                                 size_t max_shift, float coef, float *out, bool accumulate,
                                 hipStream_t s, uint32_t j0_start = 0, bool converted = false) {
    if (d == 0) return hipSuccess;
    const uint32_t nlev = bitlen(max_shift);
    if (nlev == 0) return launch_extract(src, d, coef, out, accumulate, s);
    if (L >= ((size_t)1 << 29)) return hipErrorInvalidValue;
    uint64_t *cur = src, *oth = tmp;
    for (uint32_t j0 = j0_start; j0 < nlev;) {
        const bool small = g_compact_variant == 1 || (g_compact_variant == 2 && j0 == 0);
        const uint32_t CAP = small ? 4096 : 8192;
        const uint32_t gmax = j0 == 0 ? (small ? 9 : 10) : (small ? 5 : 6);
        uint32_t G = min(gmax, nlev - j0), H = (1u << G) - 1;
        const uint64_t rows64 = (L + ((uint64_t)1 << j0) - 1) >> j0;
        const uint32_t rows = (uint32_t)rows64;
        uint32_t logW, S;
        bool nohalo = false;
        bool tail = false;
        uint32_t tcap = CAP;
        if (L <= ((size_t)1 << kCpTailMerge) && j0 > 0 && nlev - j0 > G &&
            nlev - j0 <= 10) {
            const uint32_t Gt = nlev - j0, Ht = (1u << Gt) - 1;
            const uint64_t so = (d + ((uint64_t)1 << j0) - 1) >> j0;
            auto widest = [&](uint32_t cap) {
                uint32_t lw = 0;
                while (lw < 4 && lw < j0 && ((so + Ht) << (lw + 1)) <= cap) ++lw;
                return ((so + Ht) << lw) <= cap ? (int)lw : -1;
            };
            int lw = widest(4096);
            if (lw >= 0 && lw < 4 && L > ((size_t)1 << 21) && widest(8192) >= 4) {
                lw = widest(8192);
                tcap = 8192;
            }
            if (lw >= 0 && so < rows) {
                tail = true;
                G = Gt;
                H = Ht;
                logW = (uint32_t)lw;
                S = (uint32_t)so;
            }
        }
        if (tail) {
        } else if (j0 == 0) {
            logW = 0;
            S = CAP - H;
            if (converted) S &= ~1u;
        } else {
            logW = 4;
            const bool fits = rows + H <= CAP >> logW;
            if (fits || rows <= CAP >> logW) {
                uint32_t lw = logW, lwn = logW;
                while (lw < j0 && ((rows + H) << (lw + 1)) <= CAP) ++lw;
                while (lwn < j0 && (rows << (lwn + 1)) <= CAP) ++lwn;
                if (!fits || lwn > lw) {
                    logW = lwn;
                    S = rows;
                    nohalo = true;
                } else {
                    logW = lw;
                    S = lw == 4 ? (CAP >> 4) - H : rows;
                }
            } else {
                S = (CAP >> logW) - H;
            }
            if (logW > j0) logW = j0;
        }
        const uint32_t ngroups = (uint32_t)(((uint64_t)1 << j0) >> logW);
        const uint64_t bands = tail ? 1 : (rows + S - 1) / S;
        uint64_t ntiles = bands * ngroups;
        if (ntiles == 0 || ntiles > 0x7FFFFFFFull) return hipErrorInvalidValue;
        const bool last = (j0 + G == nlev);
        const int fin = last ? (accumulate ? 2 : 1) : 0;
        uint64_t live = ntiles;
        if (last && bands == 1 && j0 > 0 && ((uint64_t)1 << j0) >= d) {
            const uint64_t g = (d + ((uint64_t)1 << logW) - 1) >> logW;
            if (g < live) live = g;
        }
        net_account(tail ? (uint64_t)8 * L + 4 * (uint64_t)d : (uint64_t)(last ? 8 : 16) * L * live / ntiles,
                    "compact_pass", s);
        ntiles = live;
        const int blk = j0 == 0 ? kCompactFirstBlocks : kCompactBlocks;
        const bool wide = tail ? tcap > 4096 : !small;
        const unsigned res = !wide ? 256u * (unsigned)blk : 256u;
        const unsigned grid = (unsigned)(ntiles < res ? ntiles : res);
        const hipError_t e =
            !wide ? launch_pass<512, 8, 8>(j0 == 0 && !converted, fin, grid, s, cur, oth, (uint32_t)L,
                                           (uint32_t)d, j0, G, logW, S, rows, ngroups, coef, out,
                                           (uint32_t)ntiles, nohalo)
                  : launch_pass<1024, 8>(j0 == 0 && !converted, fin, grid, s, cur, oth, (uint32_t)L, (uint32_t)d, j0,
                                         G, logW, S, rows, ngroups, coef, out, (uint32_t)ntiles);
        if (e != hipSuccess) return e;
        uint64_t *x = cur; cur = oth; oth = x;
        j0 += G;
    }
    return hipSuccess;
}

uint64_t compact_dummy() { return CP_DUMMY; }

hipError_t launch_compact_extract_converted(uint64_t *src, uint64_t *tmp, size_t L, size_t d,
                                            float coef, float *out, bool accumulate, hipStream_t s) {
    return compact_levels(src, tmp, L, d, L > d ? L - d : 0, coef, out, accumulate, s, 0, true);
}

hipError_t launch_compact_extract(uint64_t *src, uint64_t *tmp, size_t L, size_t d, float coef,
                                  float *out, bool accumulate, hipStream_t s) {
    return compact_levels(src, tmp, L, d, L > d ? L - d : 0, coef, out, accumulate, s);
}

constexpr int kFcBlocks = 2;
constexpr uint32_t kFixedWalkMax = 128;
constexpr uint32_t kFixedWalkMaxSmall = 320;
constexpr uint32_t kFcTilesPerCu = 1;
constexpr uint32_t kFcSpinMax = 1u << 20;

struct FcLb {
    uint64_t agg[3], inc[3];
};

__device__ __forceinline__ void fc_put(uint64_t *w, const FoldAgg &g, uint32_t epoch) {
    const uint64_t tag = (uint64_t)((epoch << 2) | (g.fl & 3u)) << 32;
    __hip_atomic_store(&w[0], tag | g.F, __ATOMIC_RELAXED, __HIP_MEMORY_SCOPE_AGENT);
    __hip_atomic_store(&w[1], tag | g.K, __ATOMIC_RELAXED, __HIP_MEMORY_SCOPE_AGENT);
    __hip_atomic_store(&w[2], tag | __float_as_uint(g.Q), __ATOMIC_RELAXED, __HIP_MEMORY_SCOPE_AGENT);
}
__device__ __forceinline__ FoldAgg fa_shfl_up(const FoldAgg &x, int o) {
    FoldAgg r;
    r.F = (uint32_t)__shfl_up((int)x.F, o);
    r.K = (uint32_t)__shfl_up((int)x.K, o);
    r.Q = __shfl_up(x.Q, o);
    r.fl = (uint32_t)__shfl_up((int)x.fl, o);
    return r;
}
__device__ __forceinline__ FoldAgg fa_shfl_down(const FoldAgg &x, int o) {
    FoldAgg r;
    r.F = (uint32_t)__shfl_down((int)x.F, o);
    r.K = (uint32_t)__shfl_down((int)x.K, o);
    r.Q = __shfl_down(x.Q, o);
    r.fl = (uint32_t)__shfl_down((int)x.fl, o);
    return r;
}

__device__ __forceinline__ bool fc_have(const uint64_t *w, uint32_t epoch, FoldAgg &g) {
    g.F = (uint32_t)w[0];
    g.K = (uint32_t)w[1];
    g.Q = __uint_as_float((uint32_t)w[2]);
    g.fl = (uint32_t)(w[2] >> 32) & 3u;
    return (uint32_t)(w[0] >> 34) == epoch && (uint32_t)(w[1] >> 34) == epoch &&
           (uint32_t)(w[2] >> 34) == epoch;
}

template <int NW>
__device__ FoldAgg fc_lookback(FcLb *lb, uint32_t tile, uint32_t epoch, uint32_t t,
                               uint32_t *status, FoldAgg *sh, uint32_t *shf, const uint64_t *pre) {
    const uint32_t lane = t & 63, wave = t >> 6;
    long long base = (long long)tile - 1;
    bool done = tile == 0;
    if (t == 0) sh[NW] = fa_empty();
    __syncthreads();
    while (!done) {
        const long long p = base - (long long)(wave * 64 + lane);
        bool isinc = true;
        FoldAgg v = fa_empty();
        if (p >= 0) {
            FoldAgg g;
            bool ok = false;
            uint32_t it = 0;
            if (base == (long long)tile - 1) {
                if (fc_have(pre, epoch, g)) { isinc = true; ok = true; }
                else if (fc_have(pre + 3, epoch, g)) { isinc = false; ok = true; }
            }
#pragma unroll 1
            while (!ok) {
                uint64_t w[6];
#pragma unroll
                for (int i = 0; i < 3; ++i) {
                    w[i] = __hip_atomic_load(&lb[p].inc[i], __ATOMIC_RELAXED, __HIP_MEMORY_SCOPE_AGENT);
                    w[3 + i] = __hip_atomic_load(&lb[p].agg[i], __ATOMIC_RELAXED, __HIP_MEMORY_SCOPE_AGENT);
                }
                if (fc_have(w, epoch, g)) { isinc = true; ok = true; break; }
                if (fc_have(w + 3, epoch, g)) { isinc = false; ok = true; break; }
                if (++it >= kFcSpinMax) break;
                __builtin_amdgcn_s_sleep(8);
            }
            if (!ok) {
                atomicOr(status, FLTEE_DEV_ERR_LAUNCH);
                g = fa_empty();
                isinc = true;
            }
            v = g;
        }
        const uint64_t incl = __ballot(isinc);
        const uint32_t first = incl ? (uint32_t)__builtin_ctzll(incl) : 64u;
        if (lane > first) v = fa_empty();
#pragma unroll
        for (int o = 1; o < 64; o <<= 1) {
            const FoldAgg older = fa_shfl_down(v, o);
            if ((lane & (2 * o - 1)) == 0) v = fa_combine(older, v);
        }
        if (lane == 0) {
            sh[wave] = v;
            shf[wave] = first < 64;
        }
        __syncthreads();
        if (t == 0) {
            FoldAgg blk = fa_empty();
            uint32_t found = 0;
#pragma unroll 1
            for (int w = 0; w < NW && !found; ++w) {
                blk = fa_combine(sh[w], blk);
                found = shf[w];
            }
            sh[NW] = fa_combine(blk, sh[NW]);
            shf[NW] = found;
        }
        __syncthreads();
        done = shf[NW] != 0;
        base -= 64 * NW;
    }
    const FoldAgg run = sh[NW];
    __syncthreads();
    return run;
}

template <int NT, int PER, int FINAL, int XMAX>
__global__ __launch_bounds__(NT, kFcBlocks * NT >= 1024 ? kFcBlocks * NT / 256 : 1) void fold_compact_first(const uint64_t *__restrict__ A,
                                                            uint64_t *__restrict__ dst, uint32_t L,
                                                            uint32_t M, uint32_t d, uint32_t G,
                                                            uint32_t S, uint32_t Hr,
                                                            uint32_t ntiles, float coef,
                                                            float *__restrict__ out,
                                                            uint32_t lim, FcLb *lb, uint32_t epoch,
                                                            uint32_t *status) {
    constexpr uint32_t CAP = (uint32_t)NT * PER;
    constexpr int NW = NT / 64;
    extern __shared__ __attribute__((aligned(16))) uint64_t win[];
    __shared__ FoldAgg wtot[NW];
    __shared__ FoldAgg agg_s;
    __shared__ FoldAgg lb_sh[NW + 1];
    __shared__ uint32_t lb_shf[NW + 1];
    __shared__ uint32_t fix_s, kw0_s;
    const uint32_t H = (1u << G) - 1;
    const uint32_t t = threadIdx.x, lane = t & 63, wave = t >> 6;
    const uint32_t Wn = Hr + CAP + 1;
    const uint32_t chunk = (Wn + NT - 1) / NT;
    const __amdgpu_buffer_rsrc_t rs =
        __builtin_amdgcn_make_buffer_rsrc((void *)A, (short)0, (int)(M * 8u), 0x00020000);
    uint64_t pf[PER + XMAX];
    auto prefetch = [&](uint32_t tl) {
        const long long wlo = (long long)tl * S - (long long)Hr;
#pragma unroll
        for (uint32_t i = 0; i < PER + XMAX; ++i) {
            const long long p = wlo + t + i * NT;
            const bool ok = p >= 0 && p < (long long)M && t + i * NT < Wn;
            const cp_u32x2 x = __builtin_amdgcn_raw_buffer_load_b64(
                rs, (int)(ok ? (uint32_t)p * 8u : 0u), 0, 0);
            pf[i] = ok ? (((uint64_t)x.y << 32) | x.x) : CP_PAD;
        }
    };
    uint32_t tile = blockIdx.x;
    if (tile >= ntiles) return;
    for (;;) {
        prefetch(tile);
        const long long a = (long long)tile * S, wlo = a - (long long)Hr;
#pragma unroll
        for (uint32_t i = 0; i < PER + XMAX; ++i)
            if (t + i * NT < Wn) win[t + i * NT] = pf[i];
        __syncthreads();
        const uint32_t next = tile + gridDim.x;
        float *sums = reinterpret_cast<float *>(win + Wn);
        const int x0 = (int)(t * chunk), ys = x0 - (int)lim;
        FoldAgg ca = fa_empty();
        float qS = 0.0f;
        {
            const int pw = (int)wlo;
            auto rd = [&](int y) { return win[min((uint32_t)max(y, 0), Wn - 1)]; };
            uint32_t prevk = 0xFFFFFFFFu;
            bool have = false;
            float acc = 0.0f;
            auto step = [&](uint64_t r, int y) {
                const uint32_t p = (uint32_t)(pw + y);
                const bool valid = ((uint32_t)y < Wn) & (p < L);
                const uint32_t ky = (uint32_t)r;
                const bool cont = have & valid & (p != 0u) & (ky == prevk);
                const float v = rec_val(r);
                acc = cont ? __fadd_rn(acc, v) : v;
                prevk = ky;
                have = valid;
            };
            uint64_t rn = rd(ys);
            for (uint32_t q = 0; q < lim; ++q) {
                const uint64_t r = rn;
                rn = rd(ys + (int)q + 1);
                step(r, ys + (int)q);
            }
            uint32_t kl = 0;
            float acc2 = 0.0f;
            bool unb = true;
            for (uint32_t i = 0; i < chunk; ++i) {
                const int y = x0 + (int)i;
                const uint64_t r = rn;
                rn = rd(y + 1);
                step(r, y);
                const bool in = y < (int)Wn;
                const uint32_t ky = (uint32_t)r;
                const bool c2 = i > 0 && ky == kl;
                acc2 = in ? (c2 ? __fadd_rn(acc2, rec_val(r)) : rec_val(r)) : acc2;
                qS = y == (int)S - 1 ? acc2 : qS;
                unb = unb && (!in || i == 0 || c2);
                kl = in ? ky : kl;
                if (in) {
                    sums[y] = acc;
                }
            }
            if (x0 < (int)Wn) {
                ca.F = (uint32_t)win[x0];
                ca.K = kl;
                ca.Q = acc2;
                ca.fl = kFsPiece | (unb ? kFsFull : 0u);
            }
        }
        FoldAgg inc = ca;
#pragma unroll
        for (int o = 1; o < 64; o <<= 1) {
            const FoldAgg y = fa_shfl_up(inc, o);
            if (lane >= (uint32_t)o) inc = fa_combine(y, inc);
        }
        FoldAgg wex = fa_shfl_up(inc, 1);
        if (lane == 0) wex = fa_empty();
        if (lane == 63) wtot[wave] = inc;
        __syncthreads();
        {
            FoldAgg ex = fa_empty();
            for (uint32_t w = 0; w < wave; ++w) ex = fa_combine(ex, wtot[w]);
            ex = fa_combine(ex, wex);
            const uint32_t k0 = x0 < (int)Wn ? (uint32_t)win[x0] : 0u;
            const bool exf = (ex.fl & kFsPiece) && ex.K == k0;
            if (t == 0) {
                fix_s = 0xFFFFFFFFu;
                kw0_s = (uint32_t)win[0];
            }
            if ((uint32_t)x0 <= S - 1 && S - 1 < (uint32_t)x0 + chunk) {
                const uint32_t kS = (uint32_t)win[S - 1];
                FoldAgg part;
                part.F = k0;
                part.K = kS;
                part.Q = qS;
                part.fl = kFsPiece | (k0 == kS ? kFsFull : 0u);
                const FoldAgg g = fa_combine(ex, part);
                fc_put(lb[tile].agg, g, epoch);
                agg_s = g;
            }
            const bool lngL = ys > 0 && x0 < (int)Wn && (uint32_t)win[ys - 1] == k0;
            float a2 = 0.0f;
            for (uint32_t i = 0; i < chunk; ++i) {
                const int y = x0 + (int)i;
                const uint64_t r = win[min(y, (int)Wn - 1)];
                a2 = i == 0 ? rec_val(r) : __fadd_rn(a2, rec_val(r));
                const bool fix = lngL && y < (int)Wn && (uint32_t)r == k0;
                if (fix) sums[y] = exf ? __fadd_rn(ex.Q, a2) : a2;
            }
        }
        __syncthreads();
        uint64_t v[PER];
        {
            const uint32_t kw0 = (uint32_t)win[0];
            const uint32_t gm = (1u << G) - 1;
#pragma unroll
            for (uint32_t i = 0; i < PER; ++i) {
                const uint32_t f = t + i * NT, x = f + Hr;
                const long long p = a + f;
                const uint64_t r = win[x];
                const uint32_t idx = (uint32_t)r;
                const bool end = p == (long long)L - 1 || (uint32_t)win[x + 1] != idx;
                const float hv = sums[x];
                const bool rep = p < (long long)L && idx < d && end;
                const uint32_t c = (uint32_t)p - idx;
                v[i] = rep ? (((uint64_t)__float_as_uint(hv) << 32) | c) : CP_DUMMY;
                if (rep && idx == kw0) fix_s = f - (c & gm);
            }
        }
        __syncthreads();
        uint64_t *sm = win;
#pragma unroll
        for (uint32_t i = 0; i < PER; ++i) sm[t + i * NT] = v[i];
        const uint64_t lw[6] = {0, 0, 0, 0, 0, 0};
        __syncthreads();
        bool lv_done = false;
        if (G == 9 && S + H == CAP) {
            cp_levels_ct<NT, PER, 9, 0, (int)CAP>(sm, 0u, t);
            lv_done = true;
        }
        uint64_t nv[PER];
        for (uint32_t g = 0; g < (lv_done ? 0u : G);) {
            const uint32_t stepf = 1u << g;
            const bool two = g + 1 < G;
            const uint32_t gl = two ? g + 1 : g;
            const uint32_t lmt = S + H - ((2u << gl) - 1);
            if (two) {
#pragma unroll
                for (uint32_t i = 0; i < PER; ++i) {
                    const uint32_t f = t + i * NT;
                    if (f < lmt) {
                        const uint64_t y0 = cp_pick(sm[f], sm[f + stepf], g);
                        const uint64_t y2 = cp_pick(sm[f + 2 * stepf], sm[f + 3 * stepf], g);
                        nv[i] = cp_pick(y0, y2, g + 1);
                    }
                }
            } else {
#pragma unroll
                for (uint32_t i = 0; i < PER; ++i) {
                    const uint32_t f = t + i * NT;
                    if (f < lmt) nv[i] = cp_pick(sm[f], sm[f + stepf], g);
                }
            }
            __syncthreads();
#pragma unroll
            for (uint32_t i = 0; i < PER; ++i) {
                const uint32_t f = t + i * NT;
                if (f < lmt) sm[f] = nv[i];
            }
            __syncthreads();
            g += two ? 2 : 1;
        }
        const FoldAgg wc = fc_lookback<NW>(lb, tile, epoch, t, status, lb_sh, lb_shf, lw);
        if (t == 0) fc_put(lb[tile].inc, fa_combine(wc, agg_s), epoch);
        const bool wok = (wc.fl & kFsPiece) && wc.K == kw0_s;
        const uint32_t fx = fix_s;
#pragma unroll
        for (uint32_t i = 0; i < PER; ++i) {
            const uint32_t f = t + i * NT;
            if (f < S) {
                const long long p = a + f;
                uint64_t rv = sm[f];
                const float fv = __fadd_rn(wc.Q, rec_val(rv));
                rv = (wok && f == fx) ? ((rv & 0xFFFFFFFFull) | ((uint64_t)__float_as_uint(fv) << 32)) : rv;
                if (FINAL == 0) {
                    if (p < (long long)L) dst[p] = rv;
                } else if (p < (long long)d) {
                    const float vv = cp_out(rv);
                    out[p] = FINAL == 2 ? __fadd_rn(out[p], vv) : __fmul_rn(vv, coef);
                }
            }
        }
        if (next >= ntiles) break;
        __syncthreads();
        tile = next;
    }
}

static bool g_fold_compact = true;
void set_fold_compact(int on) { g_fold_compact = on != 0; }

template <int PER, int F, int X>
static hipError_t fc_launch(uint64_t ntiles, size_t lds, hipStream_t s, const uint64_t *A, uint64_t *B,
                            size_t L, size_t M, size_t d, uint32_t G, uint32_t S, size_t Hr,
                            float coef, float *out, uint32_t lim, FcLb *lb, uint32_t epoch,
                            uint32_t *status) {
    constexpr int NT = 512;
    auto kern = fold_compact_first<NT, PER, F, X>;
    static int resident = 0;
    static size_t res_lds = 0;
    if (!resident || res_lds != lds) {
        (void)hipFuncSetAttribute((const void *)kern, hipFuncAttributeMaxDynamicSharedMemorySize,
                                  80 * 1024);
        int dev = 0, cus = 0, per_cu = 0;
        if (hipGetDevice(&dev) != hipSuccess ||
            hipDeviceGetAttribute(&cus, hipDeviceAttributeMultiprocessorCount, dev) != hipSuccess ||
            hipOccupancyMaxActiveBlocksPerMultiprocessor(&per_cu, (const void *)kern, NT, lds) !=
                hipSuccess)
            return hipErrorLaunchFailure;
        if (per_cu > kFcBlocks) per_cu = kFcBlocks;
        resident = (per_cu > 0 ? per_cu : 1) * (cus > 0 ? cus : 1);
        res_lds = lds;
    }
    const unsigned grid = (unsigned)(ntiles < (uint64_t)resident ? ntiles : (uint64_t)resident);
    FLTEE_LAUNCH(kern, dim3(grid), dim3(NT), lds, s, A, B, (uint32_t)L, (uint32_t)M,
                       (uint32_t)d, G, S, (uint32_t)Hr, (uint32_t)ntiles, coef, out, lim, lb, epoch,
                       status);
    return hipGetLastError();
}

template <int PER>
static hipError_t fc_dispatch(int F, bool x1, uint64_t ntiles, size_t lds, hipStream_t s,
                              const uint64_t *A, uint64_t *B, size_t L, size_t M, size_t d,
                              uint32_t G, uint32_t S, size_t Hr, float coef, float *out,
                              uint32_t lim, FcLb *lb, uint32_t epoch, uint32_t *status) {
#define FC_ARGS ntiles, lds, s, A, B, L, M, d, G, S, Hr, coef, out, lim, lb, epoch, status
    if (F == 0) return x1 ? fc_launch<PER, 0, 1>(FC_ARGS) : fc_launch<PER, 0, 2>(FC_ARGS);
    if (F == 2) return x1 ? fc_launch<PER, 2, 1>(FC_ARGS) : fc_launch<PER, 2, 2>(FC_ARGS);
    return x1 ? fc_launch<PER, 1, 1>(FC_ARGS) : fc_launch<PER, 1, 2>(FC_ARGS);
#undef FC_ARGS
}

struct FcShape {
    uint32_t per, G, S, lim;
    size_t Hr, ntiles;
};
static bool fc_shape(size_t M, size_t L, size_t d, size_t halo, FcShape &o) {
    constexpr uint32_t NT = 512;
    o.Hr = fold_context(halo + 1);
    o.lim = halo + 1 >= 0xFFFFFFFFull ? 0xFFFFFFFFu : (uint32_t)(halo + 1);
    if (!g_fold_compact || d == 0 || L <= d || o.Hr + 1 > 2 * 512 || M >= ((size_t)1 << 29) || L > M)
        return false;
    if (o.lim > kFixedWalkMax && !(o.lim <= kFixedWalkMaxSmall && M <= ((size_t)1 << 20)))
        return false;
    const uint32_t nlev = bitlen(L - d);
    o.G = nlev < 9 ? nlev : 9;
    const uint32_t H = (1u << o.G) - 1;
    o.per = 8;
    for (uint32_t p : {4u, 6u}) {
        if (NT * p <= 2 * H) continue;
        if ((L + NT * p - H - 1) / (NT * p - H) <= 256 * kFcTilesPerCu) {
            o.per = p;
            break;
        }
    }
    const uint32_t CAP = NT * o.per;
    o.S = CAP - H;
    o.ntiles = (L + o.S - 1) / o.S;
    const size_t lds = (o.Hr + CAP + 1) * 12;
    return lds * kFcBlocks <= 160 * 1024 && lds <= 80 * 1024;
}

bool fold_compact_geometry(size_t M, size_t L, size_t d, size_t halo, uint64_t out[7]) {
    FcShape o;
    if (!fc_shape(M, L, d, halo, o)) return false;
    out[0] = o.per;
    out[1] = o.S;
    out[2] = o.ntiles;
    out[3] = o.lim;
    out[4] = o.G;
    out[5] = o.G == bitlen(L - d);
    out[6] = o.Hr;
    return true;
}

size_t fc_lookback_bytes(size_t M, size_t L, size_t d, size_t halo) {
    FcShape o;
    return fc_shape(M, L, d, halo, o) ? o.ntiles * sizeof(FcLb) : 0;
}

hipError_t launch_fold_compact_extract(uint64_t *A, uint64_t *B, size_t M, size_t L, size_t d,
                                       size_t halo, float coef, float *out, bool accumulate,
                                       uint32_t *status, hipStream_t s, void *lb, size_t lb_cap,
                                       uint32_t *epoch) {
    constexpr uint32_t NT = 512;
    FcShape o;
    if (!fc_shape(M, L, d, halo, o)) return hipErrorNotSupported;
    if (!lb || lb_cap < o.ntiles * sizeof(FcLb) || !epoch) return hipErrorInvalidValue;
    if (++*epoch >= (1u << 30)) return hipErrorInvalidValue;
    const uint32_t nlev = bitlen(L - d);
    const uint32_t CAP = NT * o.per;
    const bool last = o.G == nlev;
    const size_t lds = (o.Hr + CAP + 1) * 12;
    net_account((uint64_t)(last ? 8 : 16) * L, "fold_compact_first", s);
    const bool x1 = o.Hr + 1 <= NT;
    const int F = !last ? 0 : (accumulate ? 2 : 1);
    FcLb *l = (FcLb *)lb;
    hipError_t e;
#define FC_GO(P_) fc_dispatch<P_>(F, x1, o.ntiles, lds, s, A, B, L, M, d, o.G, o.S, o.Hr, coef, out, \
                                  o.lim, l, *epoch, status)
    if (o.per == 4) e = FC_GO(4);
    else if (o.per == 6) e = FC_GO(6);
    else e = FC_GO(8);
#undef FC_GO
    if (e != hipSuccess || last) return e;
    return compact_levels(B, A, L, d, L - d, coef, out, accumulate, s, o.G);
}

__global__ void offset_copy_kernel(const uint64_t *__restrict__ chunk, size_t c, size_t d,
                                   uint64_t *__restrict__ buf) {
    const size_t L = d + c;
    for (size_t p = (size_t)blockIdx.x * 256 + threadIdx.x; p < L; p += (size_t)gridDim.x * 256)
        buf[p] = p < d ? CP_DUMMY : chunk[p - d];
}

hipError_t launch_compact_offset(const uint64_t *chunk, size_t c, size_t d, uint64_t *buf,
                                 uint64_t *tmp, float coef, float *out, hipStream_t s) {
    if (d == 0) return hipSuccess;
    const size_t L = d + c;
    if (L >= ((size_t)1 << 29)) return hipErrorInvalidValue;
    size_t blocks = (L + 255) / 256;
    if (blocks > 65536) blocks = 65536;
    FLTEE_LAUNCH(offset_copy_kernel, dim3((unsigned)blocks), dim3(256), 0, s, chunk, c, d,
                       buf);
    const hipError_t e = hipGetLastError();
    if (e != hipSuccess) return e;
    return compact_levels(buf, tmp, L, d, L - 1, coef, out, false, s);
}

}
```

### fl-tee_amd/fltee/_lib.py

```python
import ctypes
import os

PKG_ROOT = os.path.dirname(os.path.dirname(os.path.abspath(__file__)))
LIB_PATH = os.environ.get("FLTEE_LIB") or os.path.join(PKG_ROOT, "lib", "libfltee_agg.so")

SUCCESS = 0x0
ERROR_UNEXPECTED = 0x1
ERROR_INVALID_PARAMETER = 0x2
ERROR_OUT_OF_MEMORY = 0x3
ERROR_INVALID_ENCLAVE_ID = 0x2002
ERROR_MAC_MISMATCH = 0x3001

ALG_ADVANCED, ALG_NIPS19, ALG_BASELINE, ALG_NON_OBLIVIOUS, ALG_PATH_ORAM, ALG_OPTIMIZED = 1, 2, 3, 4, 5, 6
ALG_BUBBLE = 7
ALG_CODES = {
    "advanced": ALG_ADVANCED, "nips19": ALG_NIPS19, "baseline": ALG_BASELINE,
    "non_oblivious": ALG_NON_OBLIVIOUS, "path_oram": ALG_PATH_ORAM, "optimized": ALG_OPTIMIZED,
}

DEV_ERR_DENSE_ORDER = 0x1
DEV_ERR_INDEX_RANGE = 0x2
DEV_ERR_FOLD_OVERFLOW = 0x4
DEV_ERR_AUTH = 0x10

GCM_SEGMENT_BLOCKS = 512
GCM_TAG_BYTES = 16
GCM_MAX_AAD = 64
AEAD_ABORT, AEAD_REPORT, AEAD_DROP = 0, 1, 2

OPT_DENSE = 0x1
OPT_DP = 0x2
OPT_CLIP = 0x4
OPT_ACCUMULATE = 0x8
OPT_NO_AVERAGE = 0x10
OPT_K_REQ = 0x20
OPT_ORAM_TREE = 0x40
OPT_ORAM_LAZY = 0x80
OPT_PACKED = 0x100
OPT_TRIM = 0x200
TRIM_MAX = 64
AAD_PACKED_BIT = 0x80000000
OPT_BF16 = 0x400
AAD_BF16_BIT = 0x40000000


class DeviceOpts(ctypes.Structure):
    _fields_ = [
        ("flags", ctypes.c_uint32),
        ("sigma", ctypes.c_float),
        ("clipping", ctypes.c_float),
        ("seed", ctypes.c_uint64),
        ("k_req", ctypes.c_size_t),
        ("batch", ctypes.c_size_t),
        ("n_avg", ctypes.c_size_t),
        ("fold_halo", ctypes.c_size_t),
        ("d_status", ctypes.c_void_p),
        ("trim", ctypes.c_size_t),
    ]


_P, _S, _U32, _U64, _F, _U8 = (ctypes.c_void_p, ctypes.c_size_t, ctypes.c_uint32,
                               ctypes.c_uint64, ctypes.c_float, ctypes.c_uint8)
SIGNATURES = {
    "fltee_device_init": (_U32, [ctypes.c_int, _P]),
    "fltee_device_fini": (_U32, [_U64]),
    "ecall_fl_init": (_U32, [_U64, _P, _U32, _P, _S, _S, _S, _F, _F, _F, _F, _U32, _U8, _U8]),
    "ecall_start_round": (_U32, [_U64, _P, _U32, _U32, _S, _P]),
    "ecall_secure_aggregation": (_U32, [_U64, _P, _U32, _U32, _P, _S, _P, _S, _S, _S, _U32, _P, _P]),
    "ecall_client_size_optimized_secure_aggregation":
        (_U32, [_U64, _P, _U32, _U32, _S, _P, _S, _P, _S, _S, _U32, _P, _P]),
    "fltee_aggregate_device": (_U32, [_U32, _P, _S, _S, _S, _P, ctypes.POINTER(DeviceOpts), _P]),
    "fltee_workspace_bytes": (_S, [_U32, _S, _S, _S, ctypes.POINTER(DeviceOpts)]),
    "fltee_reserve": (_U32, [_U32, _S, _S, _S, ctypes.POINTER(DeviceOpts)]),
    "fltee_decrypt_device": (_U32, [_P, _S, _P, _S, _P, _P]),
    "fltee_decrypt_auth_device": (_U32, [_P, _S, _P, _S, _P, _P, _S, _P, _P, _P]),
    "fltee_encrypt_auth_device": (_U32, [_P, _S, _P, _S, _P, _P, _S, _P, _P]),
    "fltee_debug_gcm_tag_host": (_U32, [_U32, _P, _P, _S, _P, _S, _P]),
    "fltee_gcm_segments": (_S, [_S, _S]),
    "fltee_ghash_window_device": (_U32, [_P, _S, _P, _S, _S, _S, _S, _P, _S, ctypes.c_int, _P, _P]),
    "fltee_ghash_merge_device": (_U32, [_P, _P, _S, _S, _P]),
    "fltee_gcm_finish_device": (_U32, [_P, _S, _P, _S, _P, _S, _P, _P, _P]),
    "fltee_decrypt_slice_auth_device": (_U32, [_P, _S, _P, _S, _S, _S, _P, _P, _P]),
    "fltee_debug_ghash_window_host": (_U32, [_U32, _P, _S, ctypes.c_int, _P, _S, _S, _S, _P]),
    "fltee_packed_slice_bytes": (_S, [_S]),
    "fltee_upload_is_packed": (ctypes.c_int, [ctypes.c_int, _S, _S, _S]),
    "fltee_set_upload_packed": (None, [ctypes.c_int]),
    "fltee_unpack_dense_device": (_U32, [_P, _S, _S, _P, _P]),
    "fltee_client_pack_dense_device": (_U32, [_P, _S, _S, _P, _P]),
    "fltee_trim_count": (_S, [_S, _U32]),
    "fltee_set_dense_trim": (None, [_U32]),
    "fltee_bf16_slice_bytes": (_S, [_S]),
    "fltee_upload_is_bf16": (ctypes.c_int, [ctypes.c_int, _S, _S, _S]),
    "fltee_set_upload_bf16": (None, [ctypes.c_int]),
    "fltee_unpack_bf16_device": (_U32, [_P, _S, _S, _P, _P]),
    "fltee_client_pack_bf16_device": (_U32, [_P, _S, _S, _P, _P]),
    "fltee_set_upload_aead": (None, [ctypes.c_int]),
    "fltee_set_upload_aead_policy": (None, [ctypes.c_int, _S]),
    "fltee_auth_report": (_U32, [_U64, _U32, _P, _P, _S, _P]),
    "fltee_gather_clients_device": (_U32, [_P, _S, _S, _P, _S, _P, _P]),
    "fltee_device_status": (_U32, [_P, _P]),
    "fltee_sum_rows_device": (_U32, [_P, _S, _S, _F, _P, _P]),
    "fltee_dp_noise_device": (_U32, [_P, _S, _F, _F, _S, _U64, _P]),
    "fltee_bitonic_device": (_U32, [_P, _S, _U32, _U32, _P]),
    "fltee_stable_sort_device": (_U32, [_P, _S, _P]),
    "fltee_fold_device": (_U32, [_P, _P, _S, _S, _S, _P, _P]),
    "fltee_laplace_r_device": (_U32, [_S, _S, _S, _U64, _P, _P, _P]),
    "fltee_client_topk_device": (_U32, [_P, _S, _S, _S, _P, _P]),
    "fltee_client_serialize_dense_device": (_U32, [_P, _S, _S, _P, _P]),
    "fltee_client_clip_device": (_U32, [_P, _S, _S, _F, _P]),
    "fltee_encrypt_device": (_U32, [_P, _S, _P, _S, _P, _P]),
    "fltee_advanced_init_range_device": (_U32, [_P, _S, _S, _S, _S, _P, _P]),
    "fltee_bitonic_range_sort_device": (_U32, [_P, _S, _S, _U32, _U32, _P]),
    "fltee_bitonic_range_sort_padded_device": (_U32, [_P, _S, _S, _S, _U32, _U32, _P]),
    "fltee_bitonic_range_merge_device": (_U32, [_P, _S, _S, _U32, _U32, _U32, _P]),
    "fltee_bitonic_range_exchange_device": (_U32, [_P, _P, _S, _S, _S, _U32, _U32, _U32, _P]),
    "fltee_bitonic_range_steps_device": (_U32, [_P, _S, _S, _U32, _U32, _U32, _U32, _U32, _P]),
    "fltee_stable_init_range_device": (_U32, [_P, _S, _S, _S, _S, _P, _P]),
    "fltee_stable_range_sort_device": (_U32, [_P, _S, _S, _S, _P]),
    "fltee_stable_range_exchange_device": (_U32, [_P, _P, _S, _S, _S, _U32, _P]),
    "fltee_stable_range_merge_device": (_U32, [_P, _S, _S, _U32, _P]),
    "fltee_stable_range_strip_device": (_U32, [_P, _S, _P, _P]),
    "fltee_fold_context": (_S, [_S]),
    "fltee_fold_side_bytes": (_S, [_S, _S]),
    "fltee_fold_range_device": (_U32, [_P, _P, _S, _S, _S, ctypes.c_int64, _S, _S, _P, _P]),
    "fltee_fold_range_total_device": (_U32, [_P, _S, _S, _P, _P]),
    "fltee_fold_range_patch_device": (_U32, [_P, _S, _S, ctypes.c_int64, _S, _S, _P, _P, _S, _P]),
    "fltee_compact_range_device": (_U32, [_P, _S, _S, _P, _P, _F, _P, _P]),
    "fltee_nips19_build_range_device": (_U32, [_P, _S, _P, _S, _S, _S, _S, _P, _P]),
    "fltee_safe_aggregate_device": (_U32, [_P, _S, _S, _P, _P]),
    "fltee_select_device": (_U32, [_P, _S, _S, _P, _S, _P, _P]),
    "fltee_ordered_list_device": (_U32, [_P, _S, _S, _F, _P, _P]),
    "fltee_debug_sort_records_device": (_U32, [_P, _S, _S, _P, _P]),
    "fltee_debug_set_seed": (None, [_U64]),
    "fltee_set_path_oram_tree": (None, [ctypes.c_int]),
    "fltee_set_advanced_exact_runs": (None, [ctypes.c_int]),
    "fltee_set_bubble_ecall": (None, [ctypes.c_int]),
    "fltee_version": (ctypes.c_char_p, []),
    "fltee_device_init_multi": (_U32, [_P, ctypes.c_int, _P]),
    "fltee_device_count": (ctypes.c_int, [_U64]),
}
EXTRA_SIGNATURES = {
    "fltee_debug_aes_block": (None, [_P, _P, _P]),
    "fltee_debug_gf128_mul": (None, [_P, _P, _P]),
    "fltee_debug_gcm_subkeys": (ctypes.c_int, [_U32, _P, _P, ctypes.c_int]),
    "fltee_debug_gcm_segment_blocks": (_S, []),
    "fltee_debug_set_dense_variant": (None, [ctypes.c_int]),
    "fltee_debug_set_oram_bucket": (None, [ctypes.c_int]),
    "fltee_debug_set_aes_variant": (None, [ctypes.c_int]),
    "fltee_debug_read_floor": (ctypes.c_int, [_P, _S, _P, ctypes.c_uint, _P]),
    "fltee_debug_network_plan": (_S, [_U32, _U32, _U32, ctypes.c_int, _P, _S]),
    "fltee_debug_pad_units": (None, [_U32] * 8 + [_P]),
    "fltee_debug_set_advanced_compaction": (None, [ctypes.c_int]),
    "fltee_debug_set_compact_variant": (None, [ctypes.c_int]),
    "fltee_debug_set_fused_init": (None, [ctypes.c_int]),
    "fltee_debug_set_nips19_fused_select": (None, [ctypes.c_int]),
    "fltee_debug_net_stats": (None, [_P, _P, ctypes.c_int]),
    "fltee_debug_net_timing": (None, [ctypes.c_int, _P]),
    "fltee_debug_session_round_keys": (ctypes.c_int, [_P, _S, _P, ctypes.c_int]),
    "fltee_debug_net_log": (_S, [_S, ctypes.c_char_p, _S, _P, _P]),
    "fltee_debug_set_fold_compact": (None, [ctypes.c_int]),
    "fltee_debug_fold_geometry": (None, [_S, _S, _S, _S, _P]),
    "fltee_debug_plan": (_U32, [_U32, _S, _S, _S, ctypes.POINTER(DeviceOpts), _P]),
    "fltee_debug_scratch_grown": (_U32, []),
    "fltee_debug_scratch_release": (None, []),
    "fltee_debug_set_pad_skip": (None, [ctypes.c_int]),
    "fltee_debug_set_radix_order": (None, [ctypes.c_int]),
    "fltee_debug_set_swizzle": (None, [ctypes.c_int]),
    "fltee_debug_sort_fused": (_U32, [_U32, _P, _S, _P, _S, _P, _S, _S,
                                       _U32, _P]),
}

_lib = None


def lib():
    global _lib
    if _lib is None:
        if not os.path.exists(LIB_PATH):
            raise RuntimeError(
                f"{LIB_PATH} is missing: build it with `make -C {PKG_ROOT}` "
                "(the aggregation path has no CPU fallback)")
        L = ctypes.CDLL(LIB_PATH, mode=ctypes.RTLD_GLOBAL)
        ab = bool(os.environ.get("FLTEE_LIB"))
        for name, (res, args) in {**SIGNATURES, **EXTRA_SIGNATURES}.items():
            if ab and not hasattr(L, name):
                continue
            fn = getattr(L, name)
            fn.restype = res
            fn.argtypes = args
        _lib = L
    return _lib
```

Baseline: 819.4 billion client-params/s.

## Replace decoupled lookback in fold-compact with carry scan and inline carry apply

The fused fold-compact kernel used to chain tiles through a spin-wait decoupled lookback with epoch-tagged atomics. It now writes per-tile aggregates, and the cross-tile carry is resolved either inline at the start of the next compact pass (small tile counts) or by a separate single-block scan plus an apply kernel. This removes the inter-block spin dependency and the epoch and memset management. In exchange it adds an extra pass over the data or a serial per-block chain computation. The workload runs the baseline dense route, which likely does not touch this path.

Result: slower. 809.5 billion client-params/s (-1.2%).

```diff
diff --git a/fl-tee_amd/csrc/common.h b/fl-tee_amd/csrc/common.h
--- a/fl-tee_amd/csrc/common.h
+++ b/fl-tee_amd/csrc/common.h
@@ -251,11 +251,10 @@
                        uint64_t cdummy = 0);
 hipError_t launch_extract(const uint64_t *src, size_t d, float coef, float *out, bool accumulate,
                           hipStream_t s);
-size_t fc_lookback_bytes(size_t M, size_t L, size_t d, size_t halo);
+size_t fc_carry_bytes(size_t M, size_t L, size_t d, size_t halo);
 hipError_t launch_fold_compact_extract(uint64_t *A, uint64_t *B, size_t M, size_t L, size_t d,
                                        size_t halo, float coef, float *out, bool accumulate,
-                                       uint32_t *status, hipStream_t s, void *lb, size_t lb_cap,
-                                       uint32_t *epoch);
+                                       hipStream_t s, void *ws, size_t ws_cap);
 hipError_t launch_compact_extract(uint64_t *src, uint64_t *tmp, size_t L, size_t d, float coef,
                                   float *out, bool accumulate, hipStream_t s);
 uint64_t compact_dummy();
diff --git a/fl-tee_amd/csrc/engine.h b/fl-tee_amd/csrc/engine.h
--- a/fl-tee_amd/csrc/engine.h
+++ b/fl-tee_amd/csrc/engine.h
@@ -97,7 +97,6 @@
     Buffer ws_side;
     Buffer ws_lb;
     Buffer ws_s16;
-    uint32_t fc_epoch = 0;
     uint32_t *host_word = nullptr;
     hipStream_t stream = nullptr;
     hipStream_t copy_stream = nullptr;
diff --git a/fl-tee_amd/csrc/engine.hip b/fl-tee_amd/csrc/engine.hip
--- a/fl-tee_amd/csrc/engine.hip
+++ b/fl-tee_amd/csrc/engine.hip
@@ -185,7 +185,7 @@
     a.fold_len = n * k_req + d, a.halo = halo ? halo : n, a.span = a.M;
     if (a.fold_len != a.L || !g_advanced_compaction) {
         a.tail = kTailSort;
-    } else if ((a.lb_bytes = fc_lookback_bytes(a.M, a.L, d, a.halo)) != 0) {
+    } else if ((a.lb_bytes = fc_carry_bytes(a.M, a.L, d, a.halo)) != 0) {
         a.tail = kTailFused;
     } else {
         a.span = advanced_fold_span(a.L, a.M);
@@ -300,20 +300,10 @@
     return p;
 }
 
-static bool reserve_lb(DeviceCtx *c, size_t bytes, const hipStream_t *s) {
-    const bool grow = bytes > c->ws_lb.cap;
-    if (!bytes || (!grow && (!s || c->fc_epoch < (1u << 30) - 1))) return true;
-    if (!c->ws_lb.reserve(bytes)) return false;
-    if ((s ? fl_memset_async(c->ws_lb.ptr, 0, c->ws_lb.cap, *s) : fl_memset(c->ws_lb.ptr, 0, c->ws_lb.cap)) !=
-        hipSuccess)
-        return false;
-    c->fc_epoch = 0;
-    return true;
-}
-
 static bool reserve_plan(DeviceCtx *c, const Plan &p, const hipStream_t *s) {
+    (void)s;
     for (int w = 0; w < kWsCount; ++w)
-        if (!(w == kWsLb ? reserve_lb(c, p.bytes[w], s) : (c->*kScratch[w]).reserve(p.bytes[w]))) return false;
+        if (!(c->*kScratch[w]).reserve(p.bytes[w])) return false;
     return true;
 }
 
@@ -443,9 +433,8 @@
     if (e != hipSuccess) return e;
     switch (a.tail) {
     case kTailFused:
-        if (!reserve_lb(c, a.lb_bytes, &s)) return hipErrorOutOfMemory;
-        return launch_fold_compact_extract(A, B, a.M, a.L, a.d, a.halo, coef, out, acc, status, s,
-                                           c->ws_lb.ptr, c->ws_lb.cap, &c->fc_epoch);
+        return launch_fold_compact_extract(A, B, a.M, a.L, a.d, a.halo, coef, out, acc, s, c->ws_lb.ptr,
+                                           c->ws_lb.cap);
     case kTailStream:
         e = launch_fold(A, B, a.span, a.fold_len, a.halo, c->ws_side.ptr, c->ws_side.cap, s, a.d,
                         compact_dummy());
@@ -635,7 +624,6 @@
     for (auto w : kScratch) (c->*w).release();
     c->mat_clean = c->mat_clean_cap = 0;
     c->mat_clean_ptr = nullptr;
-    c->fc_epoch = 0;
 }
 
 
@@ -1137,6 +1125,7 @@
 
 namespace fltee {
 void set_dense_variant(int v); void set_compact_variant(int v); void set_fold_compact(int on);
+void set_fold_carry(int separate); void set_fold_tiles_per_block(uint32_t n);
 bool fold_compact_geometry(size_t M, size_t L, size_t d, size_t halo, uint64_t out[7]);
 bool fold_stream_geometry(size_t span, size_t fold_len, size_t halo, uint64_t out[5]);
 hipError_t launch_read_floor(const void *src, size_t bytes, uint32_t *sink, unsigned blocks, hipStream_t s);
@@ -1150,6 +1139,8 @@
 extern "C" void fltee_debug_set_advanced_compaction(int on) { fltee::g_advanced_compaction = on != 0; }
 extern "C" void fltee_debug_set_compact_variant(int v) { fltee::set_compact_variant(v); }
 extern "C" void fltee_debug_set_fold_compact(int on) { fltee::set_fold_compact(on); }
+extern "C" void fltee_debug_set_fold_carry(int separate) { fltee::set_fold_carry(separate); }
+extern "C" void fltee_debug_set_fold_tiles_per_block(unsigned n) { fltee::set_fold_tiles_per_block(n); }
 extern "C" void fltee_debug_set_pad_skip(int on) { fltee::set_pad_skip(on); }
 extern "C" void fltee_debug_set_radix_order(int on) { fltee::set_radix_order(on); }
 extern "C" void fltee_set_path_oram_tree(int on) {
diff --git a/fl-tee_amd/csrc/k_compact.hip b/fl-tee_amd/csrc/k_compact.hip
--- a/fl-tee_amd/csrc/k_compact.hip
+++ b/fl-tee_amd/csrc/k_compact.hip
@@ -60,6 +60,78 @@
     }
 }
 
+struct FcCarry {
+    uint32_t key;
+    float q;
+};
+constexpr uint32_t kFcNoKey = 0xFFFFFFFFu;
+constexpr uint32_t kFcCarryInline = 512;
+constexpr uint32_t kFcG = 9;
+
+__device__ __forceinline__ FoldAgg fa_shfl_up(const FoldAgg &x, int o) {
+    FoldAgg r;
+    r.F = (uint32_t)__shfl_up((int)x.F, o);
+    r.K = (uint32_t)__shfl_up((int)x.K, o);
+    r.Q = __shfl_up(x.Q, o);
+    r.fl = (uint32_t)__shfl_up((int)x.fl, o);
+    return r;
+}
+
+struct FcAggIn {
+    uint4 me;
+    uint32_t kprev;
+};
+__device__ __forceinline__ FcAggIn fc_carry_load(const FoldAgg *__restrict__ agg, uint32_t g) {
+    const uint4 *a4 = reinterpret_cast<const uint4 *>(agg);
+    FcAggIn r;
+    r.me = a4[g];
+    r.kprev = g ? a4[g - 1].y : kFcNoKey;
+    return r;
+}
+__device__ __forceinline__ void fc_carry_put(const FcAggIn &a, uint32_t g, uint32_t j, uint32_t *key,
+                                             float *sQ, uint32_t *sC) {
+    key[j] = (g != 0 && a.kprev == a.me.x) ? a.me.x : kFcNoKey;
+    sQ[j] = __uint_as_float(a.me.z);
+    sC[j] = (g != 0 && (a.me.w & kFsFull) && a.me.x == a.kprev) ? 0xFFFFFFFFu : 0u;
+}
+constexpr uint32_t kFcChainPad = 16;
+__device__ __forceinline__ float fc_carry_chain(float *__restrict__ cq, const float *__restrict__ sQ,
+                                                const uint32_t *__restrict__ sC, uint32_t n, float q0) {
+    const float4 *q4 = reinterpret_cast<const float4 *>(sQ);
+    const uint4 *c4 = reinterpret_cast<const uint4 *>(sC);
+    float4 *o4 = reinterpret_cast<float4 *>(cq);
+    float q = q0;
+    for (uint32_t r = 0; r < (n + 15) / 16; ++r) {
+        float x[16], o[16];
+        uint32_t c[16];
+#pragma unroll
+        for (int i = 0; i < 4; ++i) {
+            const float4 xv = q4[4 * r + i];
+            const uint4 cv = c4[4 * r + i];
+            x[4 * i] = xv.x, x[4 * i + 1] = xv.y, x[4 * i + 2] = xv.z, x[4 * i + 3] = xv.w;
+            c[4 * i] = cv.x, c[4 * i + 1] = cv.y, c[4 * i + 2] = cv.z, c[4 * i + 3] = cv.w;
+        }
+#pragma unroll
+        for (int i = 0; i < 16; ++i) {
+            o[i] = q;
+            const uint32_t qin = (__float_as_uint(q) & c[i]) | (~c[i] & 0x80000000u);
+            q = __fadd_rn(__uint_as_float(qin), x[i]);
+        }
+#pragma unroll
+        for (int i = 0; i < 4; ++i)
+            o4[4 * r + i] = make_float4(o[4 * i], o[4 * i + 1], o[4 * i + 2], o[4 * i + 3]);
+    }
+    return q;
+}
+
+__device__ __forceinline__ uint64_t fc_carry_rec(uint64_t rv, uint32_t q, const FcCarry cy, uint32_t G) {
+    const uint32_t c = (uint32_t)rv;
+    const uint32_t idx = q - (c >> G << G);
+    const bool hit = !(c >> 31) && idx == cy.key;
+    const float fv = __fadd_rn(cy.q, rec_val(rv));
+    return hit ? ((rv & 0xFFFFFFFFull) | ((uint64_t)__float_as_uint(fv) << 32)) : rv;
+}
+
 template <int NT, int PER, bool FIRST, int FINAL, int MINB = 1, bool V2 = false, int CG = 0, int CLW = 0,
           int CSH = 0, bool NH = false>
 __global__ __launch_bounds__(NT, MINB) void compact_pass(const uint64_t *__restrict__ src,
@@ -67,9 +139,15 @@
                                                    uint32_t d, uint32_t j0, uint32_t G,
                                                    uint32_t logW, uint32_t S, uint32_t rows,
                                                    uint32_t ngroups, float coef,
-                                                   float *__restrict__ out, uint32_t ntiles) {
+                                                   float *__restrict__ out, uint32_t ntiles,
+                                                   const FoldAgg *__restrict__ cagg, uint32_t cn,
+                                                   uint64_t cmul) {
     constexpr uint32_t CAP = (uint32_t)NT * PER;
-    __shared__ uint64_t sm[CAP];
+    __shared__ __attribute__((aligned(16))) uint64_t sm[CAP];
+    constexpr uint32_t CTN = (!FIRST && NT == 512 && CAP <= 4096) ? kFcCarryInline : 1;
+    __shared__ uint32_t ckey[CTN];
+    __shared__ __attribute__((aligned(16))) float ccq[CTN + kFcChainPad];
+    const bool carry = CTN > 1 && cagg != nullptr;
     const uint32_t W = 1u << logW, H = (1u << G) - 1;
     auto tid = [] {
         uint32_t x = threadIdx.x;
@@ -111,11 +189,29 @@
             }
         }
     };
-    prefetch(tile);
+    if (carry) {
+        float *sQ = reinterpret_cast<float *>(sm);
+        uint32_t *sC = reinterpret_cast<uint32_t *>(sm) + kFcCarryInline + kFcChainPad;
+        const uint32_t g = tid() < cn ? tid() : 0u;
+        const FcAggIn a = fc_carry_load(cagg, g);
+        prefetch(tile);
+        if (tid() < cn) fc_carry_put(a, g, g, ckey, sQ, sC);
+        __syncthreads();
+        if (tid() == 0) fc_carry_chain(ccq, sQ, sC, cn, 0.0f);
+        __syncthreads();
+    } else {
+        prefetch(tile);
+    }
     for (;;) {
 #pragma unroll
         for (uint32_t i = 0; i < PER; ++i) {
             uint64_t v = pos_of(tile, slot(i)) < L ? pf[i] : CP_DUMMY;
+            if (carry) {
+                const uint32_t q = (uint32_t)pos_of(tile, slot(i));
+                const uint32_t T = (uint32_t)(((uint64_t)q * cmul) >> 45);
+                const uint32_t Tc = T < cn ? T : cn - 1;
+                v = fc_carry_rec(v, q, FcCarry{ckey[Tc], ccq[Tc]}, kFcG);
+            }
             if (FIRST) {
                 const uint32_t p = (uint32_t)pos_of(tile, tid() + i * NT), idx = (uint32_t)v;
                 v = (v & 0xFFFFFFFF00000000ull) | (idx < d ? (uint64_t)(p - idx) : CP_DUMMY);
@@ -213,13 +309,14 @@
 static hipError_t launch_pass(bool first, int fin, unsigned grid, hipStream_t s, const uint64_t *src,
                               uint64_t *dst, uint32_t L, uint32_t d, uint32_t j0, uint32_t G,
                               uint32_t logW, uint32_t S, uint32_t rows, uint32_t ngroups,
-                              float coef, float *out, uint32_t ntiles, bool nh = false) {
+                              float coef, float *out, uint32_t ntiles, bool nh = false,
+                              const FoldAgg *cagg = nullptr, uint32_t cn = 0, uint64_t cmul = 0) {
 #define CP_GO(F, X, V)                                                                           \
     FLTEE_LAUNCH((compact_pass<NT, PER, F, X, MINB, V>), dim3(grid), dim3(NT), 0, s, src, dst, L, \
-                       d, j0, G, logW, S, rows, ngroups, coef, out, ntiles)
+                       d, j0, G, logW, S, rows, ngroups, coef, out, ntiles, cagg, cn, cmul)
 #define CP_GO_CT(V, G_, LW_, SH_)                                                                \
     FLTEE_LAUNCH((compact_pass<NT, PER, false, 0, MINB, V, G_, LW_, SH_>), dim3(grid), dim3(NT), 0, s, \
-                       src, dst, L, d, j0, G, logW, S, rows, ngroups, coef, out, ntiles)
+                       src, dst, L, d, j0, G, logW, S, rows, ngroups, coef, out, ntiles, cagg, cn, cmul)
     const bool v2 = !first && (logW >= 1 || S % 2 == 0) && L % 2 == 0 &&
                     (uintptr_t)src % 16 == 0 && (uintptr_t)dst % 16 == 0;
     const uint32_t sh = S + (1u << G) - 1;
@@ -231,7 +328,7 @@
     }
 #define CP_GO_NH(X, V)                                                                           \
     FLTEE_LAUNCH((compact_pass<NT, PER, false, X, MINB, V, 0, 0, 0, true>), dim3(grid), dim3(NT), 0, s, \
-                       src, dst, L, d, j0, G, logW, S, rows, ngroups, coef, out, ntiles)
+                       src, dst, L, d, j0, G, logW, S, rows, ngroups, coef, out, ntiles, cagg, cn, cmul)
     if (nh && !first) {
         if (v2) {
             if (fin == 0) CP_GO_NH(0, true); else if (fin == 1) CP_GO_NH(1, true); else CP_GO_NH(2, true);
@@ -261,7 +358,9 @@
 
 static hipError_t compact_levels(uint64_t *src, uint64_t *tmp, size_t L, size_t d,
                                  size_t max_shift, float coef, float *out, bool accumulate,
-                                 hipStream_t s, uint32_t j0_start = 0, bool converted = false) {
+                                 hipStream_t s, uint32_t j0_start = 0, bool converted = false,
+                                 const FoldAgg *cagg = nullptr, uint32_t cn = 0, uint32_t cS = 0) {
+    const uint64_t cmul = cagg ? (((uint64_t)1 << 45) + cS - 1) / cS : 0;
     if (d == 0) return hipSuccess;
     const uint32_t nlev = bitlen(max_shift);
     if (nlev == 0) return launch_extract(src, d, coef, out, accumulate, s);
@@ -343,10 +442,12 @@
         const bool wide = tail ? tcap > 4096 : !small;
         const unsigned res = !wide ? 256u * (unsigned)blk : 256u;
         const unsigned grid = (unsigned)(ntiles < res ? ntiles : res);
+        const bool cy = cagg && j0 == j0_start;
+        if (cy && (wide || cn > kFcCarryInline)) return hipErrorInvalidValue;
         const hipError_t e =
             !wide ? launch_pass<512, 8, 8>(j0 == 0 && !converted, fin, grid, s, cur, oth, (uint32_t)L,
                                            (uint32_t)d, j0, G, logW, S, rows, ngroups, coef, out,
-                                           (uint32_t)ntiles, nohalo)
+                                           (uint32_t)ntiles, nohalo, cy ? cagg : nullptr, cn, cmul)
                   : launch_pass<1024, 8>(j0 == 0 && !converted, fin, grid, s, cur, oth, (uint32_t)L, (uint32_t)d, j0,
                                          G, logW, S, rows, ngroups, coef, out, (uint32_t)ntiles);
         if (e != hipSuccess) return e;
@@ -372,134 +473,17 @@
 constexpr uint32_t kFixedWalkMax = 128;
 constexpr uint32_t kFixedWalkMaxSmall = 320;
 constexpr uint32_t kFcTilesPerCu = 1;
-constexpr uint32_t kFcSpinMax = 1u << 20;
-
-struct FcLb {
-    uint64_t agg[3], inc[3];
-};
-
-__device__ __forceinline__ void fc_put(uint64_t *w, const FoldAgg &g, uint32_t epoch) {
-    const uint64_t tag = (uint64_t)((epoch << 2) | (g.fl & 3u)) << 32;
-    __hip_atomic_store(&w[0], tag | g.F, __ATOMIC_RELAXED, __HIP_MEMORY_SCOPE_AGENT);
-    __hip_atomic_store(&w[1], tag | g.K, __ATOMIC_RELAXED, __HIP_MEMORY_SCOPE_AGENT);
-    __hip_atomic_store(&w[2], tag | __float_as_uint(g.Q), __ATOMIC_RELAXED, __HIP_MEMORY_SCOPE_AGENT);
-}
-__device__ __forceinline__ FoldAgg fa_shfl_up(const FoldAgg &x, int o) {
-    FoldAgg r;
-    r.F = (uint32_t)__shfl_up((int)x.F, o);
-    r.K = (uint32_t)__shfl_up((int)x.K, o);
-    r.Q = __shfl_up(x.Q, o);
-    r.fl = (uint32_t)__shfl_up((int)x.fl, o);
-    return r;
-}
-__device__ __forceinline__ FoldAgg fa_shfl_down(const FoldAgg &x, int o) {
-    FoldAgg r;
-    r.F = (uint32_t)__shfl_down((int)x.F, o);
-    r.K = (uint32_t)__shfl_down((int)x.K, o);
-    r.Q = __shfl_down(x.Q, o);
-    r.fl = (uint32_t)__shfl_down((int)x.fl, o);
-    return r;
-}
-
-__device__ __forceinline__ bool fc_have(const uint64_t *w, uint32_t epoch, FoldAgg &g) {
-    g.F = (uint32_t)w[0];
-    g.K = (uint32_t)w[1];
-    g.Q = __uint_as_float((uint32_t)w[2]);
-    g.fl = (uint32_t)(w[2] >> 32) & 3u;
-    return (uint32_t)(w[0] >> 34) == epoch && (uint32_t)(w[1] >> 34) == epoch &&
-           (uint32_t)(w[2] >> 34) == epoch;
-}
-
-template <int NW>
-__device__ FoldAgg fc_lookback(FcLb *lb, uint32_t tile, uint32_t epoch, uint32_t t,
-                               uint32_t *status, FoldAgg *sh, uint32_t *shf, const uint64_t *pre) {
-    const uint32_t lane = t & 63, wave = t >> 6;
-    long long base = (long long)tile - 1;
-    bool done = tile == 0;
-    if (t == 0) sh[NW] = fa_empty();
-    __syncthreads();
-    while (!done) {
-        const long long p = base - (long long)(wave * 64 + lane);
-        bool isinc = true;
-        FoldAgg v = fa_empty();
-        if (p >= 0) {
-            FoldAgg g;
-            bool ok = false;
-            uint32_t it = 0;
-            if (base == (long long)tile - 1) {
-                if (fc_have(pre, epoch, g)) { isinc = true; ok = true; }
-                else if (fc_have(pre + 3, epoch, g)) { isinc = false; ok = true; }
-            }
-#pragma unroll 1
-            while (!ok) {
-                uint64_t w[6];
-#pragma unroll
-                for (int i = 0; i < 3; ++i) {
-                    w[i] = __hip_atomic_load(&lb[p].inc[i], __ATOMIC_RELAXED, __HIP_MEMORY_SCOPE_AGENT);
-                    w[3 + i] = __hip_atomic_load(&lb[p].agg[i], __ATOMIC_RELAXED, __HIP_MEMORY_SCOPE_AGENT);
-                }
-                if (fc_have(w, epoch, g)) { isinc = true; ok = true; break; }
-                if (fc_have(w + 3, epoch, g)) { isinc = false; ok = true; break; }
-                if (++it >= kFcSpinMax) break;
-                __builtin_amdgcn_s_sleep(8);
-            }
-            if (!ok) {
-                atomicOr(status, FLTEE_DEV_ERR_LAUNCH);
-                g = fa_empty();
-                isinc = true;
-            }
-            v = g;
-        }
-        const uint64_t incl = __ballot(isinc);
-        const uint32_t first = incl ? (uint32_t)__builtin_ctzll(incl) : 64u;
-        if (lane > first) v = fa_empty();
-#pragma unroll
-        for (int o = 1; o < 64; o <<= 1) {
-            const FoldAgg older = fa_shfl_down(v, o);
-            if ((lane & (2 * o - 1)) == 0) v = fa_combine(older, v);
-        }
-        if (lane == 0) {
-            sh[wave] = v;
-            shf[wave] = first < 64;
-        }
-        __syncthreads();
-        if (t == 0) {
-            FoldAgg blk = fa_empty();
-            uint32_t found = 0;
-#pragma unroll 1
-            for (int w = 0; w < NW && !found; ++w) {
-                blk = fa_combine(sh[w], blk);
-                found = shf[w];
-            }
-            sh[NW] = fa_combine(blk, sh[NW]);
-            shf[NW] = found;
-        }
-        __syncthreads();
-        done = shf[NW] != 0;
-        base -= 64 * NW;
-    }
-    const FoldAgg run = sh[NW];
-    __syncthreads();
-    return run;
-}
-
-template <int NT, int PER, int FINAL, int XMAX>
+template <int NT, int PER, int XMAX>
 __global__ __launch_bounds__(NT, kFcBlocks * NT >= 1024 ? kFcBlocks * NT / 256 : 1) void fold_compact_first(const uint64_t *__restrict__ A,
                                                             uint64_t *__restrict__ dst, uint32_t L,
                                                             uint32_t M, uint32_t d, uint32_t G,
                                                             uint32_t S, uint32_t Hr,
-                                                            uint32_t ntiles, float coef,
-                                                            float *__restrict__ out,
-                                                            uint32_t lim, FcLb *lb, uint32_t epoch,
-                                                            uint32_t *status) {
+                                                            uint32_t ntiles, uint32_t lim,
+                                                            FoldAgg *__restrict__ agg) {
     constexpr uint32_t CAP = (uint32_t)NT * PER;
     constexpr int NW = NT / 64;
     extern __shared__ __attribute__((aligned(16))) uint64_t win[];
     __shared__ FoldAgg wtot[NW];
-    __shared__ FoldAgg agg_s;
-    __shared__ FoldAgg lb_sh[NW + 1];
-    __shared__ uint32_t lb_shf[NW + 1];
-    __shared__ uint32_t fix_s, kw0_s;
     const uint32_t H = (1u << G) - 1;
     const uint32_t t = threadIdx.x, lane = t & 63, wave = t >> 6;
     const uint32_t Wn = Hr + CAP + 1;
@@ -596,10 +580,6 @@
             ex = fa_combine(ex, wex);
             const uint32_t k0 = x0 < (int)Wn ? (uint32_t)win[x0] : 0u;
             const bool exf = (ex.fl & kFsPiece) && ex.K == k0;
-            if (t == 0) {
-                fix_s = 0xFFFFFFFFu;
-                kw0_s = (uint32_t)win[0];
-            }
             if ((uint32_t)x0 <= S - 1 && S - 1 < (uint32_t)x0 + chunk) {
                 const uint32_t kS = (uint32_t)win[S - 1];
                 FoldAgg part;
@@ -608,8 +588,12 @@
                 part.Q = qS;
                 part.fl = kFsPiece | (k0 == kS ? kFsFull : 0u);
                 const FoldAgg g = fa_combine(ex, part);
-                fc_put(lb[tile].agg, g, epoch);
-                agg_s = g;
+                const cp_u32x4 gw = {g.F, g.K, __float_as_uint(g.Q), g.fl};
+                __builtin_amdgcn_sched_barrier(0);
+                *reinterpret_cast<cp_u32x4 *>(agg + tile) = gw;
+                __builtin_amdgcn_sched_barrier(0);
+                asm volatile("s_nop 1" ::: "memory");
+                __builtin_amdgcn_sched_barrier(0);
             }
             const bool lngL = ys > 0 && x0 < (int)Wn && (uint32_t)win[ys - 1] == k0;
             float a2 = 0.0f;
@@ -624,8 +608,6 @@
         __syncthreads();
         uint64_t v[PER];
         {
-            const uint32_t kw0 = (uint32_t)win[0];
-            const uint32_t gm = (1u << G) - 1;
 #pragma unroll
             for (uint32_t i = 0; i < PER; ++i) {
                 const uint32_t f = t + i * NT, x = f + Hr;
@@ -637,14 +619,12 @@
                 const bool rep = p < (long long)L && idx < d && end;
                 const uint32_t c = (uint32_t)p - idx;
                 v[i] = rep ? (((uint64_t)__float_as_uint(hv) << 32) | c) : CP_DUMMY;
-                if (rep && idx == kw0) fix_s = f - (c & gm);
             }
         }
         __syncthreads();
         uint64_t *sm = win;
 #pragma unroll
         for (uint32_t i = 0; i < PER; ++i) sm[t + i * NT] = v[i];
-        const uint64_t lw[6] = {0, 0, 0, 0, 0, 0};
         __syncthreads();
         bool lv_done = false;
         if (G == 9 && S + H == CAP) {
@@ -683,25 +663,10 @@
             __syncthreads();
             g += two ? 2 : 1;
         }
-        const FoldAgg wc = fc_lookback<NW>(lb, tile, epoch, t, status, lb_sh, lb_shf, lw);
-        if (t == 0) fc_put(lb[tile].inc, fa_combine(wc, agg_s), epoch);
-        const bool wok = (wc.fl & kFsPiece) && wc.K == kw0_s;
-        const uint32_t fx = fix_s;
 #pragma unroll
         for (uint32_t i = 0; i < PER; ++i) {
             const uint32_t f = t + i * NT;
-            if (f < S) {
-                const long long p = a + f;
-                uint64_t rv = sm[f];
-                const float fv = __fadd_rn(wc.Q, rec_val(rv));
-                rv = (wok && f == fx) ? ((rv & 0xFFFFFFFFull) | ((uint64_t)__float_as_uint(fv) << 32)) : rv;
-                if (FINAL == 0) {
-                    if (p < (long long)L) dst[p] = rv;
-                } else if (p < (long long)d) {
-                    const float vv = cp_out(rv);
-                    out[p] = FINAL == 2 ? __fadd_rn(out[p], vv) : __fmul_rn(vv, coef);
-                }
-            }
+            if (f < S && a + f < (long long)L) dst[a + f] = sm[f];
         }
         if (next >= ntiles) break;
         __syncthreads();
@@ -712,45 +677,77 @@
 static bool g_fold_compact = true;
 void set_fold_compact(int on) { g_fold_compact = on != 0; }
 
-template <int PER, int F, int X>
+__global__ __launch_bounds__(512) void fc_carry_scan(const FoldAgg *__restrict__ agg, uint32_t n,
+                                                     FcCarry *__restrict__ tab) {
+    __shared__ uint32_t key[512];
+    __shared__ __attribute__((aligned(16))) float cq[512 + kFcChainPad], sQ[512 + kFcChainPad];
+    __shared__ __attribute__((aligned(16))) uint32_t sC[512 + kFcChainPad];
+    __shared__ float qnext;
+    const uint32_t t = threadIdx.x;
+    float q0 = 0.0f;
+    for (uint32_t base = 0; base < n; base += 512) {
+        const uint32_t m = n - base < 512u ? n - base : 512u;
+        if (t < m) fc_carry_put(fc_carry_load(agg, base + t), base + t, t, key, sQ, sC);
+        __syncthreads();
+        if (t == 0) qnext = fc_carry_chain(cq, sQ, sC, m, q0);
+        __syncthreads();
+        if (t < m) tab[base + t] = FcCarry{key[t], cq[t]};
+        q0 = qnext;
+        __syncthreads();
+    }
+}
+
+template <int FINAL>
+__global__ __launch_bounds__(256) void fc_carry_apply(uint64_t *__restrict__ buf,
+                                                      const FcCarry *__restrict__ tab, uint32_t L,
+                                                      uint32_t d, uint32_t S, uint32_t G, float coef,
+                                                      float *__restrict__ out) {
+    const FcCarry cy = tab[blockIdx.x];
+    const uint32_t a = blockIdx.x * S;
+    for (uint32_t f = threadIdx.x; f < S; f += 256) {
+        const uint32_t p = a + f;
+        if (p >= (FINAL == 0 ? L : d)) break;
+        const uint64_t rv = fc_carry_rec(buf[p], p, cy, G);
+        if (FINAL == 0) {
+            buf[p] = rv;
+        } else {
+            const float vv = cp_out(rv);
+            out[p] = FINAL == 2 ? __fadd_rn(out[p], vv) : __fmul_rn(vv, coef);
+        }
+    }
+}
+
+static bool g_fc_carry_separate = false;
+void set_fold_carry(int separate) { g_fc_carry_separate = separate != 0; }
+static uint32_t g_fc_tiles_per_block = 0;
+void set_fold_tiles_per_block(uint32_t n) { g_fc_tiles_per_block = n; }
+
+template <int PER, int X>
 static hipError_t fc_launch(uint64_t ntiles, size_t lds, hipStream_t s, const uint64_t *A, uint64_t *B,
                             size_t L, size_t M, size_t d, uint32_t G, uint32_t S, size_t Hr,
-                            float coef, float *out, uint32_t lim, FcLb *lb, uint32_t epoch,
-                            uint32_t *status) {
+                            uint32_t lim, FoldAgg *agg) {
     constexpr int NT = 512;
-    auto kern = fold_compact_first<NT, PER, F, X>;
-    static int resident = 0;
-    static size_t res_lds = 0;
-    if (!resident || res_lds != lds) {
+    auto kern = fold_compact_first<NT, PER, X>;
+    static bool attr = false;
+    if (!attr) {
         (void)hipFuncSetAttribute((const void *)kern, hipFuncAttributeMaxDynamicSharedMemorySize,
                                   80 * 1024);
-        int dev = 0, cus = 0, per_cu = 0;
-        if (hipGetDevice(&dev) != hipSuccess ||
-            hipDeviceGetAttribute(&cus, hipDeviceAttributeMultiprocessorCount, dev) != hipSuccess ||
-            hipOccupancyMaxActiveBlocksPerMultiprocessor(&per_cu, (const void *)kern, NT, lds) !=
-                hipSuccess)
-            return hipErrorLaunchFailure;
-        if (per_cu > kFcBlocks) per_cu = kFcBlocks;
-        resident = (per_cu > 0 ? per_cu : 1) * (cus > 0 ? cus : 1);
-        res_lds = lds;
-    }
-    const unsigned grid = (unsigned)(ntiles < (uint64_t)resident ? ntiles : (uint64_t)resident);
+        attr = true;
+    }
+    const uint64_t res = g_fc_tiles_per_block ? (ntiles + g_fc_tiles_per_block - 1) / g_fc_tiles_per_block
+                                              : 256u * (uint64_t)kFcBlocks;
+    const unsigned grid = (unsigned)(ntiles < res ? ntiles : res);
     FLTEE_LAUNCH(kern, dim3(grid), dim3(NT), lds, s, A, B, (uint32_t)L, (uint32_t)M,
-                       (uint32_t)d, G, S, (uint32_t)Hr, (uint32_t)ntiles, coef, out, lim, lb, epoch,
-                       status);
+                       (uint32_t)d, G, S, (uint32_t)Hr, (uint32_t)ntiles, lim, agg);
     return hipGetLastError();
 }
 
 template <int PER>
-static hipError_t fc_dispatch(int F, bool x1, uint64_t ntiles, size_t lds, hipStream_t s,
+static hipError_t fc_dispatch(bool x1, uint64_t ntiles, size_t lds, hipStream_t s,
                               const uint64_t *A, uint64_t *B, size_t L, size_t M, size_t d,
-                              uint32_t G, uint32_t S, size_t Hr, float coef, float *out,
-                              uint32_t lim, FcLb *lb, uint32_t epoch, uint32_t *status) {
-#define FC_ARGS ntiles, lds, s, A, B, L, M, d, G, S, Hr, coef, out, lim, lb, epoch, status
-    if (F == 0) return x1 ? fc_launch<PER, 0, 1>(FC_ARGS) : fc_launch<PER, 0, 2>(FC_ARGS);
-    if (F == 2) return x1 ? fc_launch<PER, 2, 1>(FC_ARGS) : fc_launch<PER, 2, 2>(FC_ARGS);
-    return x1 ? fc_launch<PER, 1, 1>(FC_ARGS) : fc_launch<PER, 1, 2>(FC_ARGS);
-#undef FC_ARGS
+                              uint32_t G, uint32_t S, size_t Hr, uint32_t lim, FoldAgg *agg) {
+    return x1 ? fc_launch<PER, 1>(ntiles, lds, s, A, B, L, M, d, G, S, Hr, lim, agg)
+              : fc_launch<PER, 2>(ntiles, lds, s, A, B, L, M, d, G, S, Hr, lim, agg);
 }
 
 struct FcShape {
@@ -796,36 +793,45 @@
     return true;
 }
 
-size_t fc_lookback_bytes(size_t M, size_t L, size_t d, size_t halo) {
+size_t fc_carry_bytes(size_t M, size_t L, size_t d, size_t halo) {
     FcShape o;
-    return fc_shape(M, L, d, halo, o) ? o.ntiles * sizeof(FcLb) : 0;
+    return fc_shape(M, L, d, halo, o) ? o.ntiles * (sizeof(FoldAgg) + sizeof(FcCarry)) : 0;
 }
 
 hipError_t launch_fold_compact_extract(uint64_t *A, uint64_t *B, size_t M, size_t L, size_t d,
                                        size_t halo, float coef, float *out, bool accumulate,
-                                       uint32_t *status, hipStream_t s, void *lb, size_t lb_cap,
-                                       uint32_t *epoch) {
+                                       hipStream_t s, void *ws, size_t ws_cap) {
     constexpr uint32_t NT = 512;
     FcShape o;
     if (!fc_shape(M, L, d, halo, o)) return hipErrorNotSupported;
-    if (!lb || lb_cap < o.ntiles * sizeof(FcLb) || !epoch) return hipErrorInvalidValue;
-    if (++*epoch >= (1u << 30)) return hipErrorInvalidValue;
+    if (!ws || (uintptr_t)ws % 16 != 0 || ws_cap < o.ntiles * (sizeof(FoldAgg) + sizeof(FcCarry)))
+        return hipErrorInvalidValue;
     const uint32_t nlev = bitlen(L - d);
     const uint32_t CAP = NT * o.per;
     const bool last = o.G == nlev;
     const size_t lds = (o.Hr + CAP + 1) * 12;
-    net_account((uint64_t)(last ? 8 : 16) * L, "fold_compact_first", s);
+    net_account((uint64_t)16 * L, "fold_compact_first", s);
     const bool x1 = o.Hr + 1 <= NT;
-    const int F = !last ? 0 : (accumulate ? 2 : 1);
-    FcLb *l = (FcLb *)lb;
+    FoldAgg *agg = (FoldAgg *)ws;
+    FcCarry *tab = (FcCarry *)(agg + o.ntiles);
     hipError_t e;
-#define FC_GO(P_) fc_dispatch<P_>(F, x1, o.ntiles, lds, s, A, B, L, M, d, o.G, o.S, o.Hr, coef, out, \
-                                  o.lim, l, *epoch, status)
+#define FC_GO(P_) fc_dispatch<P_>(x1, o.ntiles, lds, s, A, B, L, M, d, o.G, o.S, o.Hr, o.lim, agg)
     if (o.per == 4) e = FC_GO(4);
     else if (o.per == 6) e = FC_GO(6);
     else e = FC_GO(8);
 #undef FC_GO
-    if (e != hipSuccess || last) return e;
+    if (e != hipSuccess) return e;
+    const bool inl = !last && !g_fc_carry_separate && o.ntiles <= kFcCarryInline && g_compact_variant == 1;
+    if (inl) return compact_levels(B, A, L, d, L - d, coef, out, accumulate, s, o.G, false, agg,
+                                   (uint32_t)o.ntiles, o.S);
+    FLTEE_LAUNCH(fc_carry_scan, dim3(1), dim3(512), 0, s, agg, (uint32_t)o.ntiles, tab);
+    if ((e = hipGetLastError()) != hipSuccess) return e;
+    net_account((uint64_t)(last ? 8 : 16) * L, "fc_carry_apply", s);
+    const dim3 grid((unsigned)o.ntiles), blk(256);
+    if (!last) FLTEE_LAUNCH(fc_carry_apply<0>, grid, blk, 0, s, B, tab, (uint32_t)L, (uint32_t)d, o.S, o.G, coef, out);
+    else if (accumulate) FLTEE_LAUNCH(fc_carry_apply<2>, grid, blk, 0, s, B, tab, (uint32_t)L, (uint32_t)d, o.S, o.G, coef, out);
+    else FLTEE_LAUNCH(fc_carry_apply<1>, grid, blk, 0, s, B, tab, (uint32_t)L, (uint32_t)d, o.S, o.G, coef, out);
+    if ((e = hipGetLastError()) != hipSuccess || last) return e;
     return compact_levels(B, A, L, d, L - d, coef, out, accumulate, s, o.G);
 }
 
diff --git a/fl-tee_amd/fltee/_lib.py b/fl-tee_amd/fltee/_lib.py
--- a/fl-tee_amd/fltee/_lib.py
+++ b/fl-tee_amd/fltee/_lib.py
@@ -159,6 +159,8 @@
     "fltee_debug_session_round_keys": (ctypes.c_int, [_P, _S, _P, ctypes.c_int]),
     "fltee_debug_net_log": (_S, [_S, ctypes.c_char_p, _S, _P, _P]),
     "fltee_debug_set_fold_compact": (None, [ctypes.c_int]),
+    "fltee_debug_set_fold_carry": (None, [ctypes.c_int]),
+    "fltee_debug_set_fold_tiles_per_block": (None, [ctypes.c_uint]),
     "fltee_debug_fold_geometry": (None, [_S, _S, _S, _S, _P]),
     "fltee_debug_plan": (_U32, [_U32, _S, _S, _S, ctypes.POINTER(DeviceOpts), _P]),
     "fltee_debug_scratch_grown": (_U32, []),
```
